# lux-liang/Robust-Audio-Deepfake-Evolution

Measured on AMD Instinct MI355X. Metric: Phase-6 train throughput (utterances/sec), DualStreamSEMamba + LoRA + RawBoost/codec + FGM, higher is better.
Workload: dtype fp16; 1 GPU; Phase6_Proposed.conf train step on ASVspoof19-LA-shaped utterances; micro_batch=8, accumulation=4, global_batch=32, seq_len=64600, parallelism=dp1, fgm=True, mixup=True, rawboost_algo=5, lora_mode=reference, hip_graphs=True, window_batched_clean_passes=True

## Files before the change

### include/radhip.h

```cpp
#ifndef RADHIP_H
#define RADHIP_H

#include <stdint.h>

#ifdef __cplusplus
extern "C" {
#endif

#define RDX_OK 0
#define RDX_EINVAL (-1)
#define RDX_EUNSUPPORTED (-2)

typedef enum { RDX_F32 = 0, RDX_BF16 = 1 } rdx_dtype;

const char* rdx_version(void);
const char* rdx_strerror(int code);

int rdx_sincconv_absmaxpool_fwd(const float* x, int64_t batch, int64_t len, const float* filters,
                                int channels, int ksize, int mask_lo, int mask_hi, float* out,
                                void* stream);
int rdx_sincconv_absmaxpool_fwd_devmask(const float* x, int64_t batch, int64_t len,
                                        const float* filters, int channels, int ksize,
                                        const int32_t* mask_dev, int mask_stride, float* out,
                                        void* stream);
int rdx_sincconv_absmaxpool_f16mfma(const float* x, int64_t batch, int64_t len, const float* filters, int channels,
                                    int ksize, int mask_lo, int mask_hi, const int32_t* mask_dev, int mask_stride,
                                    float* out, void* stream);
int rdx_sincconv_abspool1d_fwd(const float* x, int64_t batch, int64_t len, const float* filters,
                               int channels, int ksize, int mask_lo, int mask_hi, float* out, void* stream);


int rdx_dwconv_bidir_fwd(int dtype, const void* x, int64_t ldx, const float* w, const float* bias,
                         void* u, int B, int L, int D, int K, int dirs, void* stream);
int rdx_dwconv_bidir_bwd_parts(int L);
int rdx_dwconv_bidir_bwd(int dtype, const void* x, int64_t ldx, const float* w, const float* bias,
                         const void* du, void* dx, int64_t lddx, float* dw_part, float* db_part, int64_t ld_part,
                         int B, int L, int D, int K, int dirs, void* stream);

int64_t rdx_scan_ckpt_elems(int B, int L, int D, int N, int dirs);
int rdx_scan_nblk_d(int D);
int rdx_selective_scan_fwd(int dtype, const void* u, const void* delta, const float* A_log,
                           const void* Bm, const void* Cm, int64_t ldbc, const float* Dp,
                           const float* dt_bias, float* y, float* ckpt, int B, int L, int D, int N,
                           int dirs, void* stream);
int rdx_selective_scan_bwd(int dtype, const void* u, const void* delta, const float* A_log,
                           const void* Bm, const void* Cm, int64_t ldbc, const float* Dp,
                           const float* dt_bias, const float* ckpt, const float* dy,
                           int64_t dy_dir_stride, void* du, void* ddelta, float* dBC,
                           float* dA_part, float* dD_part, float* dbias_part, int B, int L, int D,
                           int N, int dirs, void* stream);

int rdx_bigate_fwd(int dtype, const float* y, int dirs, const void* z, int64_t ldz, void* g,
                   float* ysum, int B, int L, int D, void* stream);
int rdx_bigate_bwd(int dtype, const void* dg, const void* z, int64_t ldz, const float* ysum,
                   float* dy, void* dz, int64_t lddz, int B, int L, int D, void* stream);

int rdx_row_ln_fwd(int dtype_x, const void* x, const float* gamma, const float* beta, float eps, int dtype_y, void* y,
                   float* mean, float* rstd, int64_t M, int C, void* stream);
int rdx_row_ln_bwd(int dtype_dy, const void* dy, int dtype_x, const void* x, const float* mean, const float* rstd,
                   const float* gamma, void* dx, float* dgamma, float* dbeta, int64_t M, int C, void* stream);

int rdx_layer_wsum_fwd(int dtype, int nl, const void* const* hs, const float* w, void* out,
                       int64_t n, void* stream);
int rdx_layer_wsum_nblk(int64_t n);
int rdx_layer_wsum_bwd(int dtype, int nl, const void* const* hs, const float* w, const void* g,
                       void* const* dhs, float* dot_part, int64_t n, void* stream);
int rdx_cast_f32_many(int n, const float* const* src, void* const* dst, const int64_t* numel, void* stream);
int rdx_add_f32_many(int n, void* const* dst, const float* const* src, const int64_t* numel, int copy, void* stream);

typedef struct {
  int64_t offset;
  int64_t len;
  int32_t algo;
  int32_t n_a;
  double b[6];
  double a[6];
  double f;
  double beta;
  double snr_db;
  uint64_t seed;
} rdx_rawboost_utt;

int64_t rdx_rawboost_workspace_bytes(int nutt, int64_t total_samples);
int rdx_rawboost_batch(const float* x, float* out, const rdx_rawboost_utt* utts, int nutt,
                       void* workspace, const double* noise_isd, const double* noise_ssi,
                       void* stream);

int rdx_resample_kernel(int orig_freq, int new_freq, int lowpass_width, double rolloff,
                        float* host_kernel, int host_kernel_cap, int* width_out, int* orig_g_out,
                        int* new_g_out);
typedef struct {
  int64_t in_offset, in_len, out_offset, out_len;
  int32_t orig_g, new_g, width, kern_offset;
} rdx_resample_job;
int rdx_resample_batch(const float* in, float* out, const float* kernels,
                       const rdx_resample_job* jobs, int njobs, void* stream);

int rdx_pad_mixup(const float* sig, const int64_t* offsets, const int64_t* lens,
                  const int64_t* starts, int nutt, int64_t max_len, const int* perm, float lam,
                  float* out, void* stream);

int rdx_fgm_attack(int ntensors, float* const* params, const float* const* grads,
                   float* const* backup, const int64_t* numels, float eps, double* workspace,
                   void* stream);

int rdx_focal_mixup_fwd(const void* logits, int logits_bf16, int ld, int B, int C, const int64_t* ya,
                        const int64_t* yb, const float* lam, int rows_per_lam, float alpha, float gamma,
                        int mode, float scale, float* loss, float* dlogits, void* stream);
int rdx_focal_mixup_bwd(const float* grad, const float* dlogits, void* out, int out_bf16, int n, void* stream);

int rdx_ocsupcon_eligible(const void* feats, int ld, int R, int D, int B);
int rdx_ocsupcon_mixup_fwd(const void* feats, int feats_bf16, int ld, int R, int D, const float* center,
                           const int64_t* ya, const int64_t* yb, const float* lam, int rows_per_lam,
                           float r_real, float r_fake, float alpha, float lambda_supcon, float temperature,
                           float base_temperature, float scale, float* loss, float* loss_parts, float* dfeats,
                           float* dcenter_parts, void* stream);
int rdx_ocsupcon_mixup_bwd(const float* grad, const float* dfeats, void* out, int out_bf16, int64_t n,
                           const float* dcenter_parts, int K, int D, float* dcenter, void* stream);

int rdx_gat_eligible(const void* x, int N, int Din, int Dout, float temp);
int rdx_gat_att_fwd(const float* x, const float* W, const float* b, const float* w, float temp, int B, int N,
                    int Din, int Dout, float* att, float* agg, void* stream);
int rdx_gat_att_bwd(const float* dagg, const float* x, const float* W, const float* b, const float* w, float temp,
                    const float* att, int B, int N, int Din, int Dout, float* dx, float* dW, float* db, float* dw,
                    void* stream);

int rdx_bnselu_fwd(int dtype, const void* c, const float* conv_bias, const float* mean, const float* invstd,
                   const float* weight, const float* bias, void* y, int64_t npix, int C, void* stream);
int rdx_bnselu_bwd(int dtype, const void* c, const void* dy, const float* conv_bias, const float* mean,
                   const float* invstd, const float* weight, const float* bias, void* dc, float* sums,
                   int64_t npix, int C, void* stream);
int rdx_res_tail_fwd(int dtype, const void* a, const void* identity, const float* bias, void* y,
                     uint8_t* argmax, int64_t rows, int W, int C, void* stream);
int rdx_res_tail_bwd(int dtype, const void* dy, const uint8_t* argmax, void* dx, float* dbias, int64_t rows,
                     int W, int C, void* stream);
int rdx_sincnet_b0_fwd(const void* x, const float* w1, const float* wd, const float* bn, void* c, void* y, void* idn,
                       int N, int H, int W, int C, void* stream);
int rdx_sincnet_b0_nblk(int64_t npix);
int rdx_b0x_fwd(const void* x, const float* w1, const float* wd, const float* bn, const void* w2, const float* bias,
                void* y, uint8_t* arg, int N, int H, int W, void* stream);
int rdx_b0x_bwd_nblk(int N, int W);
int rdx_b0x_bwd(const void* x, const void* dp, const uint8_t* arg, const float* w1, const float* wd, const float* bn,
                const void* w2f, float* dx, float* part, int N, int H, int W, void* stream);
int rdx_sincnet_b0_bwd(const void* x, const void* dc, const void* di, const float* w1, const float* wd, float* dx,
                       float* part, int N, int H, int W, int C, void* stream);

int rdx_posconv_fwd(const void* h, const void* wk, const float* bias, void* y, void* u, int B, int T, void* stream);
int rdx_posconv_bwd(const void* dy, const void* u, const void* wkt, void* dh, int B, int T, void* stream);

int rdx_attn_fwd(const void* q, int64_t ldq, const void* k, int64_t ldk, const void* v, int64_t ldv,
                 const float* gate, const float* rel_bias, const int64_t* seed_dev, int salt, float p_drop,
                 float scale, void* o, int64_t ldo, float* lse, uint32_t* keep_mask, int B, int T, int H, int head_dim,
                 void* stream);
int64_t rdx_attn_keep_mask_words(int B, int T, int H);
int rdx_attn_bwd(const void* q, int64_t ldq, const void* k, int64_t ldk, const void* v, int64_t ldv,
                 const float* gate, const float* rel_bias, const int64_t* seed_dev, int salt, float p_drop, float scale,
                 const void* o, int64_t ldo, const float* lse, const void* dout, int64_t lddo, float* D, void* dq,
                 void* dk, void* dv, int64_t ldg, float* dgate, int B, int T, int H, int head_dim, void* stream);
int rdx_attn_bwd_fused(const void* q, int64_t ldq, const void* k, int64_t ldk, const void* v, int64_t ldv,
                       const float* gate, const float* rel_bias, const uint32_t* keep_mask, float p_drop, float scale,
                       const void* o, int64_t ldo, const float* lse, const void* dout, int64_t lddo, float* D,
                       void* dq, void* dk, void* dv, int64_t ldg, float* dgate, int B, int T, int H, int head_dim,
                       void* stream);
int64_t rdx_attn_bwd_split_ws(int B, int H);
int rdx_attn_bwd_fused_split(const void* q, int64_t ldq, const void* k, int64_t ldk, const void* v, int64_t ldv,
                             const float* gate, const float* rel_bias, const uint32_t* keep_mask, float p_drop,
                             float scale, const void* o, int64_t ldo, const float* lse, const void* dout,
                             int64_t lddo, float* D, void* dq, void* dk, void* dv, int64_t ldg, float* dgate,
                             float* ws, int64_t ws_floats, int* counters, int64_t n_counters, int B, int T, int H,
                             int head_dim, void* stream);
int rdx_attn_dropout_mask(const int64_t* seed_dev, int salt, float p_drop, uint8_t* keep, int64_t n, int T,
                          void* stream);
int rdx_dropout_mask(const int64_t* seed_dev, int salt, float p_drop, uint8_t* keep, int64_t n, void* stream);

int rdx_wl_ln1_fwd(const float* h, const float* gamma, const float* beta, float eps, const float* wg,
                   const float* bg, const float* gconst, const void* lora_aq, const void* lora_av, int r,
                   const int64_t* seed_dev, int salt_q, int salt_v, float p_lora, void* x1, int64_t ldx, float* gate, float* mean,
                   float* rstd, int64_t M, int E, void* stream);
int rdx_wl_add_ln_fwd(const float* h, const void* delta, const int64_t* seed_dev, int salt, float p, float* h2,
                      const float* gamma, const float* beta, float eps, void* x, float* mean, float* rstd,
                      int64_t M, int E, void* stream);
int rdx_wl_residual(const float* h, const void* delta, const int64_t* seed_dev, int salt, float p, float* out,
                    int64_t n, void* stream);
int rdx_wl_dropout_bwd(const float* g, const int64_t* seed_dev, int salt, float p, void* out, int64_t n,
                       void* stream);
int rdx_wl_gelu(int mode, const void* u, const void* dy, void* out, int64_t n, void* stream);
int rdx_wl_ln_bwd(const void* dx, int64_t ldd, const float* h, const float* mean, const float* rstd,
                  const float* gamma, const float* dres, float* dh, const int64_t* seed_dev, int salt, float p,
                  void* ddrop, int64_t M, int E, void* stream);
int rdx_wl_ln1_bwd(const void* dx1, int64_t ldx, const float* dgate, const float* h, const float* mean,
                   const float* rstd, const float* gamma, const float* beta, const float* wg, const float* bg,
                   const float* gconst, const void* lora_aq, const void* lora_av, int r,
                   const int64_t* seed_dev, int salt_q, int salt_v, float p_lora, const float* dres, float* dh, void* xd, int64_t M, int E,
                   void* stream);
int rdx_wl_res_ln1_fwd(const float* h2, const void* delta, int salt_res, float p_res, float* hout,
                       const float* gamma, const float* beta, float eps, const float* wg, const float* bg,
                       const float* gconst, const void* lora_aq, const void* lora_av, int r, const int64_t* seed_dev,
                       int salt_q, int salt_v, float p_lora, void* x1, int64_t ldx, float* gate, float* mean,
                       float* rstd, int64_t M, int E, void* stream);
int rdx_wl_ln1_bwd_ex(const void* dx1, int64_t ldx, const float* dgate, const float* h, const float* mean,
                      const float* rstd, const float* gamma, const float* beta, const float* wg, const float* bg,
                      const float* gconst, const void* lora_aq, const void* lora_av, int r, const int64_t* seed_dev,
                      int salt_q, int salt_v, float p_lora, const float* dres, float* dh, void* xd,
                      const float* state_grad, const float* state_weight, int salt_prev, float p_prev,
                      void* ddrop_prev, int64_t M, int E, void* stream);
int rdx_wl_lora_grad(const void* dqkv, int64_t ldq, const void* x1, int64_t ldx, const void* dx1, int64_t ldd,
                     const int64_t* seed_dev, int salt_q, int salt_v, float p_lora, float scale, float* daq,
                     float* dbq, float* dav, float* dbv, int64_t M, int E, int r, void* stream);
int rdx_wl_lora_pack(int nl, const float* const* bq, const float* const* bv, void* const* wext, int64_t ldw,
                     int r, float scale, int E, void* stream);

#define RDX_EPI_BIAS 0
#define RDX_EPI_BIAS_GELU 1
#define RDX_EPI_GELU_BWD 2
#define RDX_EPI_RESID_DROP 3
int rdx_gemm_bf16(const void* A, int64_t lda, const void* B, int64_t ldb, void* C, int64_t ldc, int M, int N, int K,
                  const void* bias, int epilogue, const void* aux, int64_t ldaux, void* aux_out, int64_t ldao,
                  const int64_t* seed_dev, int salt, float p_drop, void* stream);

int rdx_scan2_chunks(int L);
int64_t rdx_scan2_rec_elems(int B, int L, int D, int N, int dirs);
int rdx_scan2_fwd(int dtype, const void* u, const void* delta, const float* A_log, const void* Bm, const void* Cm,
                  int64_t ldbc, const float* Dp, const float* dt_bias, float* y, float* ckpt, float* P, float* hloc,
                  int B, int L, int D, int N, int dirs, void* stream);
int rdx_scan2_bwd(int dtype, const void* u, const void* delta, const float* A_log, const void* Bm, const void* Cm,
                  int64_t ldbc, const float* Dp, const float* dt_bias, const float* ckpt, const float* P,
                  const float* dy, int64_t dy_dir_stride, void* du, void* ddelta, float* dBC, float* dA_part,
                  float* dD_part, float* dbias_part, int64_t ld_part, float* gloc, int B, int L, int D, int N,
                  int dirs, void* stream);

int rdx_wgemm_bf16(const void* A, int64_t lda, const void* B, int64_t ldb, void* C, int64_t ldc, int M, int N, int K,
                   const void* bias, int epilogue, const void* aux, int64_t ldaux, void* aux_out, int64_t ldao,
                   int tile, void* stream);
int rdx_wgemm_pick(int M, int N, int K);
int rdx_wgemm_bf16_ex(const void* A, int64_t lda, const void* B, int64_t ldb, void* C, int64_t ldc, int M, int N,
                      int K, const void* bias, int epilogue, const void* aux, int64_t ldaux, void* aux_out,
                      int64_t ldao, int tile, int splits, void* ws, int64_t ws_bytes, int* counters,
                      int64_t n_counters, void* stream);
int64_t rdx_wgemm_ws_bytes(int M, int N, int tile, int splits);
int64_t rdx_wgemm_counters(int M, int N, int tile);

int rdx_pgemm_bf16(const void* A, int64_t lda, const void* B, int64_t ldb, void* C, int64_t ldc, int M, int N, int K,
                   const void* bias, int epilogue, const void* aux, int64_t ldaux, void* aux_out, int64_t ldao,
                   int tile, int group_m, void* stream);
int rdx_pgemm_prof(const void* A, int64_t lda, const void* B, int64_t ldb, void* C, int64_t ldc, int M, int N, int K,
                   const void* bias, int tile, int group_m, void* prof, void* stream);

int rdx_hgemm(const void* A, int64_t lda, const void* B, int64_t ldb, void* C, int64_t ldc, int M, int N, int K,
              const void* bias, int epilogue, const void* aux, int64_t ldaux, void* aux_out, int64_t ldao, int tile,
              int splits, int group_m, void* ws, int64_t ws_bytes, int* counters, int64_t n_counters, void* stream);
int64_t rdx_hgemm_ws_bytes(int M, int N, int tile, int splits);
int64_t rdx_hgemm_counters(int M, int N, int tile);
int64_t rdx_hgemm_sk_ws_bytes(int M, int N, int K, int tile);
int rdx_hgemm_batched(const void* A, int64_t lda, int64_t sa, const void* B, int64_t ldb, void* C, int64_t ldc,
                      int64_t sc, int M, int N, int K, int batch, const void* bias, int tile, int group_m, void* stream);

#define RDX_EPI_F32 4
#define RDX_EPI_F32_GELU_SPLIT 5
int rdx_hgemm_x3(const void* A, const void* A_lo, int64_t lda, int64_t sa, const void* B, const void* B_lo,
                 int64_t ldb, void* C, void* C_lo, int64_t ldc, int64_t sc, int M, int N, int K, int batch,
                 const float* bias, int epilogue, int tile, int splits, int group_m, void* ws, int64_t ws_bytes,
                 int* counters, int64_t n_counters, void* stream);

int rdx_x3_split(const float* x, int64_t ldx, int64_t rows, int cols, void* hi, void* lo, int64_t ldo, void* stream);
int rdx_x3_ln_split(const float* a, const float* b, float* sum_out, const float* gamma, const float* beta, float eps,
                    void* hi, void* lo, int64_t ldo, float* y32, const float* wg, const float* bg, const float* gconst,
                    float* gate, int64_t M, int E, void* stream);
int rdx_x3_attn_fwd(const float* q, const float* k, const float* v, int64_t ld, const float* gate, const float* rel,
                    float scaling, void* ohi, void* olo, int64_t ldo, int B, int T, int H, int qsplit, void* stream);
int rdx_x3_posconv_fwd(const float* h, const void* wk_hi, const void* wk_lo, const float* bias, float* out, int B,
                       int T, void* stream);
int rdx_x3_fe_conv0(const float* x, int64_t batch, int64_t len, const float* w, const float* bias, const float* gamma,
                    const float* beta, float eps, int ksize, int stride, void* out_hi, void* out_lo, void* stream);
int rdx_x3_fe_ln_gelu(const float* in, int64_t rows, const float* bias, const float* gamma, const float* beta,
                      float eps, void* out_hi, void* out_lo, float* out32, void* stream);

int rdx_x3_b0x_fwd(const float* x, const float* fbn, const float* w1, const float* wd, const float* bn,
                   const void* w2_hi, const void* w2_lo, const float* bias, float* y, int N, int H, int W,
                   void* stream);
int rdx_x3_sconv_fwd(const float* x, const void* w_hi, const void* w_lo, const float* bn, float* y, int N, int H,
                     int W, int ci, int co, int kh, int ph, void* stream);

int rdx_colsum_many(int n, const float* const* in, const int* rows, const int* cols, const int64_t* ld,
                    float* const* out, void* stream);

int rdx_lgemm(const void* A, int64_t lda, int a_f32, const void* W, int64_t ldw, void* C, int64_t ldc, int c_f32,
              int M, int N, int K, const void* bias, int epilogue, const void* aux, int64_t ldaux, void* aux_out,
              int64_t ldao, const void* R, int64_t ldr, void* stream);

int rdx_wgrad_chunk(int M, int N, int K);
int64_t rdx_wgrad_ws_floats(int M, int N, int K);
int rdx_wgrad_acc(const void* dy, int64_t ldy, const void* x, int64_t ldx, int M, int N, int K, float* dw, int64_t ldw,
                  float* db, float* ws, int64_t ws_floats, void* stream);
int64_t rdx_wgrad_many_ws_floats(int n, const int* M, const int* N, const int* K, const int* has_db);
int rdx_wgrad_acc_many(int n, const void* const* dy, const int64_t* ldy, const void* const* x, const int64_t* ldx,
                       const int* M, const int* N, const int* K, float* const* dw, const int64_t* ldw,
                       float* const* db, float* ws, int64_t ws_floats, void* stream);

int rdx_adamw_many_max(void);
int rdx_adamw_many(int n, float* const* params, float* const* grads, float* const* exp_avg, float* const* exp_avg_sq,
                   const float* const* step, const int64_t* numel, double lr, double beta1, double beta2,
                   double weight_decay, double eps, const float* grad_scale, const float* found_inf, void* stream);

int rdx_timestamp_acc(int64_t* acc, int sign, void* stream);
int rdx_wallclock_khz(int device);

int rdx_gemm_bf16_strided(const void* A, int64_t lda, int64_t sA, const void* B, int64_t ldb, void* C, int64_t ldc,
                          int64_t crow, int batch, int M, int N, int K, const void* bias, void* stream);

int rdx_fe_conv0(const float* x, int64_t batch, int64_t len, const float* w, const float* bias, const float* gamma,
                 const float* beta, float eps, int ksize, int stride, void* out, void* stream);
int rdx_fe_ln_gelu(void* io, int64_t rows, const float* gamma, const float* beta, float eps, float* out32,
                   void* stream);

int rdx_sconv_fwd(const void* x, const void* w, void* y, void* y2, const float* bn, int N, int H, int W, int ci,
                  int co, int kh, int ph, void* stream);
int rdx_sconv_fwd_res(const void* x, const void* w, void* y, const void* res, int N, int H, int W, int ci, int co,
                      int kh, int ph, void* stream);
int rdx_sconv_dgrad_bnselu(const void* dy, const void* w, const void* c, void* dc, const float* bn, float* sums,
                           int N, int H, int W, int ci, int co, int kh, int ph, void* stream);
int rdx_sconv_fwd_pool(const void* x, const void* w, const void* idn, const float* bias, void* y, uint8_t* arg, int N,
                       int H, int W, int ci, int co, void* stream);
int rdx_sconv_fwd_res_pool(const void* x, const void* w, void* y, const void* dp, const uint8_t* arg, float* dbias,
                           int N, int H, int W, int ci, int co, int kh, int ph, void* stream);
int rdx_sconv_dgrad_bnselu_pool(const void* dp, const uint8_t* arg, const void* w, const void* c, void* dc,
                                const float* bn, float* sums, int N, int H, int W, int ci, int co, int kh, int ph,
                                void* stream);
int rdx_sconv_dgrad_pool(const void* dp, const uint8_t* arg, const void* w, void* dx, int N, int H, int W, int ci,
                         int co, int kh, int ph, void* stream);
int rdx_sconv_wgrad_pool(const void* x, const void* dp, const uint8_t* arg, float* dw, float* part, int N, int H,
                         int W, int ci, int co, int kh, int ph, void* stream);
int rdx_sconv_wgrad_nblk(int N, int Ho, int W);
int rdx_sconv_wgrad(const void* x, const void* dy, float* dw, float* part, int N, int H, int W, int ci, int co,
                    int kh, int ph, void* stream);
int rdx_se_fwd(const void* x, const void* w1, const void* w2, void* y, void* m, void* h, void* s, int B, int T, int C,
               int R, void* stream);
int64_t rdx_se_bwd_part_floats(int B, int C, int R);
int rdx_se_bwd(const void* dy, const void* x, const void* w1, const void* w2, const void* m, const void* h, const void* s,
               void* dx, float* part, float* dw1, float* dw2, int B, int T, int C, int R, void* stream);
int rdx_attn_pool_fwd(const void* f, const void* w, const void* bias, void* feat, float* a, int B, int T, int C,
                      void* stream);
int rdx_attn_pool_bwd(const void* f, const void* w, const float* a, const void* dfeat, void* df, float* part, float* dw,
                      float* db, int B, int T, int C, void* stream);
int rdx_upcat_fwd(const void* fw, const void* fs, void* out, int B, int T1, int T2, int C, void* stream);
int rdx_upcat_bwd(const void* dout, void* dfs, int B, int T1, int T2, int C, void* stream);
int rdx_sconv_wprep_many(int n, const float* const* src, void* const* wf, void* const* wd, const int* co,
                         const int* ci, const int* kh, void* stream);

#ifdef __cplusplus
}
#endif
#endif
```

### robust-audio-deepfake-evolution_amd/csrc/wavlm_layer.hip

```cpp
#include "common.h"

namespace rdx {

constexpr int WL_E = 1024;
constexpr int WL_VPL = WL_E / RDX_WAVE;
constexpr int WL_R2 = 16;

struct Drop {
  const int64_t* seed_dev;
  int salt;
  uint32_t thr;
  float inv_keep;
};

__device__ __forceinline__ float drop_scale(const Drop& d, uint64_t seed, uint64_t idx) {
  return drop_keep(seed, idx, d.thr) ? d.inv_keep : 0.f;
}

__device__ __forceinline__ void load16(const float* p, float* v) {
  const float4* q = reinterpret_cast<const float4*>(p);
#pragma unroll
  for (int i = 0; i < 4; ++i) {
    float4 t = q[i];
    v[4 * i] = t.x; v[4 * i + 1] = t.y; v[4 * i + 2] = t.z; v[4 * i + 3] = t.w;
  }
}
__device__ __forceinline__ void store16(float* p, const float* v) {
  float4* q = reinterpret_cast<float4*>(p);
#pragma unroll
  for (int i = 0; i < 4; ++i) q[i] = make_float4(v[4 * i], v[4 * i + 1], v[4 * i + 2], v[4 * i + 3]);
}
__device__ __forceinline__ void load16_bf(const hst* p, float* v) {
  const uint4* q = reinterpret_cast<const uint4*>(p);
#pragma unroll
  for (int i = 0; i < 2; ++i) {
    uint4 t = q[i];
    uint32_t w[4] = {t.x, t.y, t.z, t.w};
#pragma unroll
    for (int j = 0; j < 4; ++j) {
      v[8 * i + 2 * j] = hlo(w[j]);
      v[8 * i + 2 * j + 1] = hhi(w[j]);
    }
  }
}
struct Bf16x16 {
  uint4 q[2];
};
__device__ __forceinline__ Bf16x16 load16_bf_raw(const hst* p) {
  const uint4* q = reinterpret_cast<const uint4*>(p);
  return Bf16x16{{q[0], q[1]}};
}
__device__ __forceinline__ void unpack16_bf(const Bf16x16& t, float* v) {
#pragma unroll
  for (int i = 0; i < 2; ++i) {
    uint32_t w[4] = {t.q[i].x, t.q[i].y, t.q[i].z, t.q[i].w};
#pragma unroll
    for (int j = 0; j < 4; ++j) {
      v[8 * i + 2 * j] = hlo(w[j]);
      v[8 * i + 2 * j + 1] = hhi(w[j]);
    }
  }
}
__device__ __forceinline__ void store16_bf(hst* p, const float* v) {
  uint4* q = reinterpret_cast<uint4*>(p);
#pragma unroll
  for (int i = 0; i < 2; ++i) {
    uint32_t w[4];
#pragma unroll
    for (int j = 0; j < 4; ++j) w[j] = hbits(v[8 * i + 2 * j]) | (hbits(v[8 * i + 2 * j + 1]) << 16);
    q[i] = make_uint4(w[0], w[1], w[2], w[3]);
  }
}

__device__ __forceinline__ void row_stats(const float* v, float eps, float& mean, float& rstd) {
  float s = 0.f;
#pragma unroll
  for (int i = 0; i < WL_VPL; ++i) s += v[i];
  mean = wave_sum(s) * (1.0f / WL_E);
  float q = 0.f;
#pragma unroll
  for (int i = 0; i < WL_VPL; ++i) {
    float d = v[i] - mean;
    q += d * d;
  }
  rstd = rsqrtf(wave_sum(q) * (1.0f / WL_E) + eps);
}

__device__ __forceinline__ float wave_sum16(float* v, int lane) {
  float w8[8], w4[4], w2[2];
  const bool h5 = lane & 32, h4 = lane & 16, h3 = lane & 8, h2 = lane & 4;
#pragma unroll
  for (int j = 0; j < 8; ++j) {
    float r = __shfl_xor(h5 ? v[j] : v[j + 8], 32, 64);
    w8[j] = (h5 ? v[j + 8] : v[j]) + r;
  }
#pragma unroll
  for (int j = 0; j < 4; ++j) {
    float r = __shfl_xor(h4 ? w8[j] : w8[j + 4], 16, 64);
    w4[j] = (h4 ? w8[j + 4] : w8[j]) + r;
  }
#pragma unroll
  for (int j = 0; j < 2; ++j) {
    float r = __shfl_xor(h3 ? w4[j] : w4[j + 2], 8, 64);
    w2[j] = (h3 ? w4[j + 2] : w4[j]) + r;
  }
  float r = __shfl_xor(h2 ? w2[0] : w2[1], 4, 64);
  float t = (h2 ? w2[1] : w2[0]) + r;
  t += __shfl_xor(t, 2, 64);
  t += __shfl_xor(t, 1, 64);
  return t;
}
__device__ __forceinline__ int sum16_index(int lane) {
  return 8 * ((lane >> 5) & 1) + 4 * ((lane >> 4) & 1) + 2 * ((lane >> 3) & 1) + ((lane >> 2) & 1);
}

struct GateW {
  const float* wg;
  const float* bg;
  const float* gconst;
};

__device__ __forceinline__ void gate_z(const GateW& g, const float* wgp, const float* x, int lane, float* z) {
  const int part = lane & 3;
#pragma unroll
  for (int j = 0; j < 8; ++j) {
    const float4* w = reinterpret_cast<const float4*>(wgp + j * 64 + part * 16);
    float acc = 0.f;
#pragma unroll
    for (int i = 0; i < 4; ++i) {
      float4 t = w[i];
      acc += t.x * x[4 * i] + t.y * x[4 * i + 1] + t.z * x[4 * i + 2] + t.w * x[4 * i + 3];
    }
    acc += __shfl_xor(acc, 1, 64);
    acc += __shfl_xor(acc, 2, 64);
    z[j] = acc + g.bg[j];
  }
}

struct Ln1Args {
  const float* h;
  const float* gamma;
  const float* beta;
  float eps;
  GateW g;
  const hst* Aq;
  const hst* Av;
  Drop dq, dv;
  hst* x1;
  int64_t ldx;
  float* gate;
  float* mean;
  float* rstd;
  int64_t M;
  const float* h2;
  const hst* delta;
  Drop dres;
  float* hout;
};

#ifndef WL_LN1_ROWS_DEF
#define WL_LN1_ROWS_DEF 4
#endif
constexpr int WL_LN1_ROWS = WL_LN1_ROWS_DEF;
constexpr int WL_LN1_THREADS = WL_LN1_ROWS * RDX_WAVE;

typedef __attribute__((ext_vector_type(4))) int wl_i32x4;
__device__ void wl_load_lds(wl_i32x4 rsrc, __attribute__((address_space(3))) uint32_t* lds, int size, int voffset,
                            int soffset, int offset, int aux) __asm("llvm.amdgcn.raw.buffer.load.lds");
__device__ __forceinline__ wl_i32x4 wl_rsrc(const void* base, uint32_t bytes) {
  const uint64_t a = (uint64_t)base;
  wl_i32x4 r;
  r.x = (int)(uint32_t)a;
  r.y = (int)(uint32_t)(a >> 32);
  r.z = (int)bytes;
  r.w = 0x00020000;
  return r;
}
constexpr int WL_A_INSTR = WL_R2 * WL_E * 2 / 1024 / (WL_LN1_THREADS / 64);
static_assert(WL_A_INSTR * 1024 * (WL_LN1_THREADS / 64) == WL_R2 * WL_E * 2, "whole 1 KB instructions per wave");
template <bool kLora>
__device__ __forceinline__ void stage_dma(float* swg, hst* sA, const float* wg, const hst* Aq, const hst* Av) {
  const int wv = __builtin_amdgcn_readfirstlane(threadIdx.x >> 6), lane = threadIdx.x & 63;
  constexpr int NW = WL_LN1_THREADS / 64;
  if (wv == 0) {
    const wl_i32x4 rg = wl_rsrc(wg, 8 * 64 * 4);
#pragma unroll
    for (int q = 0; q < 2; ++q)
      wl_load_lds(rg, (__attribute__((address_space(3))) uint32_t*)(reinterpret_cast<char*>(swg) + 1024 * q), 16,
                  1024 * q + 16 * lane, 0, 0, 0);
  }
  if (kLora) {
    const wl_i32x4 rq = wl_rsrc(Aq, WL_R2 / 2 * WL_E * 2), rv = wl_rsrc(Av, WL_R2 / 2 * WL_E * 2);
#pragma unroll
    for (int j = 0; j < WL_A_INSTR; ++j) {
      const int q = wv + NW * j;
      constexpr int half = WL_R2 / 2 * WL_E * 2 / 1024;
      wl_load_lds(j < WL_A_INSTR / 2 ? rq : rv,
                  (__attribute__((address_space(3))) uint32_t*)(reinterpret_cast<char*>(sA) + 1024 * q), 16,
                  1024 * (q % half) + 16 * lane, 0, 0, 0);
    }
  }
}

template <bool kLora>
__global__ __launch_bounds__(WL_LN1_THREADS) void wl_ln1_fwd_kernel(Ln1Args a) {
  __shared__ __attribute__((aligned(16))) hst sA[kLora ? WL_R2 * WL_E : 8];
  __shared__ __attribute__((aligned(16))) float swg[8 * 64];
  const int lane = threadIdx.x & 63;
  const int64_t m = (int64_t)blockIdx.x * WL_LN1_ROWS + (threadIdx.x >> 6);
  const bool live = m < a.M;
  const int e0 = lane * WL_VPL;
  float v[WL_VPL], gm[WL_VPL], bt[WL_VPL], dl[WL_VPL];
  Bf16x16 dlr;
  const uint64_t sr = (a.h2 && a.dres.thr) ? attn_seed(a.dres.seed_dev, a.dres.salt) : 0;
  stage_dma<kLora>(swg, sA, a.g.wg, a.Aq, a.Av);
  if (live) {
    load16(a.h2 ? a.h2 + m * WL_E + e0 : a.h + m * WL_E + e0, v);
    if (a.h2) dlr = load16_bf_raw(a.delta + m * WL_E + e0);
    load16(a.gamma + e0, gm);
    load16(a.beta + e0, bt);
  }
  __builtin_amdgcn_s_waitcnt(0);
  __syncthreads();
  if (live) {
    if (a.h2) {
      unpack16_bf(dlr, dl);

#pragma unroll
      for (int i = 0; i < WL_VPL; ++i)
        v[i] += dl[i] * (a.dres.thr ? drop_scale(a.dres, sr, (uint64_t)m * WL_E + e0 + i) : 1.0f);
      store16(a.hout + m * WL_E + e0, v);
    }
    float mean, rstd;
    row_stats(v, a.eps, mean, rstd);
#pragma unroll
    for (int i = 0; i < WL_VPL; ++i) v[i] = hround((v[i] - mean) * rstd * gm[i] + bt[i]);
    store16_bf(a.x1 + m * a.ldx + e0, v);
    if (lane == 0) {
      a.mean[m] = mean;
      a.rstd[m] = rstd;
    }
    float z[8];
    gate_z(a.g, swg, v, lane, z);
    if ((lane & 3) == 0) {
      const int head = lane >> 2;
      float ga = sigmoidf_(z[0] + z[1] + z[2] + z[3]);
      float gb = sigmoidf_(z[4] + z[5] + z[6] + z[7]);
      a.gate[m * (WL_E / 64) + head] = ga * (gb * a.g.gconst[head] - 1.0f) + 2.0f;
    }
  }
  if (kLora) {
    if (!live) return;
    const uint64_t sq = a.dq.thr ? attn_seed(a.dq.seed_dev, a.dq.salt) : 0;
    const uint64_t sv = a.dv.thr ? attn_seed(a.dv.seed_dev, a.dv.salt) : 0;
    uint32_t mq[WL_VPL / 2], mv[WL_VPL / 2];
#pragma unroll
    for (int j = 0; j < WL_VPL / 2; ++j) {
      const uint64_t idx = (uint64_t)m * WL_E + e0 + 2 * j;
      mq[j] = hpack2(v[2 * j] * drop_scale(a.dq, sq, idx), v[2 * j + 1] * drop_scale(a.dq, sq, idx + 1));
      mv[j] = hpack2(v[2 * j] * drop_scale(a.dv, sv, idx), v[2 * j + 1] * drop_scale(a.dv, sv, idx + 1));
    }
    float acc[WL_R2];
#pragma unroll
    for (int k = 0; k < WL_R2; ++k) {
      const uint32_t* x = k < WL_R2 / 2 ? mq : mv;
      const uint4* wp = reinterpret_cast<const uint4*>(sA + k * WL_E + e0);
      const uint4 w0 = wp[0], w1 = wp[1];
      const uint32_t w[8] = {w0.x, w0.y, w0.z, w0.w, w1.x, w1.y, w1.z, w1.w};
      float s = 0.f;
#pragma unroll
      for (int j = 0; j < WL_VPL / 2; ++j) s = hdot2(w[j], x[j], s);
      acc[k] = s;
    }
    float tot = wave_sum16(acc, lane);
    if ((lane & 3) == 0) a.x1[m * a.ldx + WL_E + sum16_index(lane)] = f2h(tot);
  }
}

struct AddLnArgs {
  const float* h;
  const hst* delta;
  Drop d;
  float* h2;
  const float* gamma;
  const float* beta;
  float eps;
  hst* x;
  float* mean;
  float* rstd;
  int64_t M;
};

__global__ __launch_bounds__(256) void wl_add_ln_fwd_kernel(AddLnArgs a) {
  const int lane = threadIdx.x & 63;
  const int64_t m = (int64_t)blockIdx.x * 4 + (threadIdx.x >> 6);
  if (m >= a.M) return;
  const int e0 = lane * WL_VPL;
  float v[WL_VPL], dl[WL_VPL], gm[WL_VPL], bt[WL_VPL];
  load16(a.h + m * WL_E + e0, v);
  const Bf16x16 dlr = load16_bf_raw(a.delta + m * WL_E + e0);
  load16(a.gamma + e0, gm);
  load16(a.beta + e0, bt);
  unpack16_bf(dlr, dl);
  const uint64_t seed = a.d.thr ? attn_seed(a.d.seed_dev, a.d.salt) : 0;
#pragma unroll
  for (int i = 0; i < WL_VPL; ++i)
    v[i] += dl[i] * (a.d.thr ? drop_scale(a.d, seed, (uint64_t)m * WL_E + e0 + i) : 1.0f);
  store16(a.h2 + m * WL_E + e0, v);
  float mean, rstd;
  row_stats(v, a.eps, mean, rstd);
#pragma unroll
  for (int i = 0; i < WL_VPL; ++i) v[i] = (v[i] - mean) * rstd * gm[i] + bt[i];
  store16_bf(a.x + m * WL_E + e0, v);
  if (lane == 0) {
    a.mean[m] = mean;
    a.rstd[m] = rstd;
  }
}

__global__ __launch_bounds__(256) void wl_residual_kernel(const float* __restrict__ h,
                                                          const hst* __restrict__ delta, Drop d,
                                                          float* __restrict__ out, int64_t n) {
  const int64_t i0 = ((int64_t)blockIdx.x * 256 + threadIdx.x) * 8;
  if (i0 >= n) return;
  const uint64_t seed = d.thr ? attn_seed(d.seed_dev, d.salt) : 0;
  float4 a0 = reinterpret_cast<const float4*>(h + i0)[0], a1 = reinterpret_cast<const float4*>(h + i0)[1];
  float x[8] = {a0.x, a0.y, a0.z, a0.w, a1.x, a1.y, a1.z, a1.w};
  uint4 t = *reinterpret_cast<const uint4*>(delta + i0);
  uint32_t w[4] = {t.x, t.y, t.z, t.w};
#pragma unroll
  for (int j = 0; j < 8; ++j) {
    float dv = (j & 1) ? hhi(w[j >> 1]) : hlo(w[j >> 1]);
    x[j] += dv * (d.thr ? drop_scale(d, seed, (uint64_t)(i0 + j)) : 1.0f);
  }
  reinterpret_cast<float4*>(out + i0)[0] = make_float4(x[0], x[1], x[2], x[3]);
  reinterpret_cast<float4*>(out + i0)[1] = make_float4(x[4], x[5], x[6], x[7]);
}

__global__ __launch_bounds__(256) void wl_dropout_bwd_kernel(const float* __restrict__ g, Drop d,
                                                             hst* __restrict__ out, int64_t n) {
  const int64_t i0 = ((int64_t)blockIdx.x * 256 + threadIdx.x) * 8;
  if (i0 >= n) return;
  const uint64_t seed = d.thr ? attn_seed(d.seed_dev, d.salt) : 0;
  float4 a0 = reinterpret_cast<const float4*>(g + i0)[0], a1 = reinterpret_cast<const float4*>(g + i0)[1];
  float x[8] = {a0.x, a0.y, a0.z, a0.w, a1.x, a1.y, a1.z, a1.w};
  uint32_t w[4];
#pragma unroll
  for (int j = 0; j < 4; ++j) {
    float s0 = d.thr ? drop_scale(d, seed, (uint64_t)(i0 + 2 * j)) : 1.0f;
    float s1 = d.thr ? drop_scale(d, seed, (uint64_t)(i0 + 2 * j + 1)) : 1.0f;
    w[j] = hbits(x[2 * j] * s0) | (hbits(x[2 * j + 1] * s1) << 16);
  }
  *reinterpret_cast<uint4*>(out + i0) = make_uint4(w[0], w[1], w[2], w[3]);
}

__device__ __forceinline__ float gelu_erf(float x) { return 0.5f * x * (1.0f + erff(x * 0.70710678118654752f)); }
__device__ __forceinline__ float gelu_erf_grad(float x) {
  return 0.5f * (1.0f + erff(x * 0.70710678118654752f)) + x * 0.39894228040143268f * __expf(-0.5f * x * x);
}

template <int kMode>
__global__ __launch_bounds__(256) void wl_gelu_kernel(const hst* __restrict__ u,
                                                      const hst* __restrict__ dy,
                                                      hst* __restrict__ out, int64_t n) {
  const int64_t i0 = ((int64_t)blockIdx.x * 256 + threadIdx.x) * 8;
  if (i0 >= n) return;
  uint4 t = *reinterpret_cast<const uint4*>(u + i0);
  uint32_t w[4] = {t.x, t.y, t.z, t.w}, gw[4] = {0, 0, 0, 0};
  if (kMode == 1) {
    uint4 g = *reinterpret_cast<const uint4*>(dy + i0);
    gw[0] = g.x; gw[1] = g.y; gw[2] = g.z; gw[3] = g.w;
  }
  uint32_t o[4];
#pragma unroll
  for (int j = 0; j < 4; ++j) {
    float x0 = hlo(w[j]), x1 = hhi(w[j]);
    float y0, y1;
    if (kMode == 0) {
      y0 = gelu_erf(x0);
      y1 = gelu_erf(x1);
    } else {
      y0 = hlo(gw[j]) * gelu_erf_grad(x0);
      y1 = hhi(gw[j]) * gelu_erf_grad(x1);
    }
    o[j] = hbits(y0) | (hbits(y1) << 16);
  }
  *reinterpret_cast<uint4*>(out + i0) = make_uint4(o[0], o[1], o[2], o[3]);
}

struct LnBwdArgs {
  const hst* dx;
  int64_t ldd;
  const float* h;
  const float* mean;
  const float* rstd;
  const float* gamma;
  const float* dres;
  float* dh;
  Drop d;
  hst* ddrop;
  int64_t M;
};

__device__ __forceinline__ void ln_bwd_row(const float* dx, const float* x, float mean, float rstd, const float* gm,
                                           float* out) {
  float g[WL_VPL], xh[WL_VPL], s1 = 0.f, s2 = 0.f;
#pragma unroll
  for (int i = 0; i < WL_VPL; ++i) {
    xh[i] = (x[i] - mean) * rstd;
    g[i] = dx[i] * gm[i];
    s1 += g[i];
    s2 += g[i] * xh[i];
  }
  s1 = wave_sum(s1) * (1.0f / WL_E);
  s2 = wave_sum(s2) * (1.0f / WL_E);
#pragma unroll
  for (int i = 0; i < WL_VPL; ++i) out[i] = rstd * (g[i] - s1 - xh[i] * s2);
}

__global__ __launch_bounds__(256) void wl_ln_bwd_kernel(LnBwdArgs a) {
  const int lane = threadIdx.x & 63;
  const int64_t m = (int64_t)blockIdx.x * 4 + (threadIdx.x >> 6);
  if (m >= a.M) return;
  const int e0 = lane * WL_VPL;
  float dx[WL_VPL], x[WL_VPL], gm[WL_VPL], o[WL_VPL], r[WL_VPL];
  const uint64_t seed = (a.ddrop && a.d.thr) ? attn_seed(a.d.seed_dev, a.d.salt) : 0;
  const Bf16x16 dxr = load16_bf_raw(a.dx + m * a.ldd + e0);
  load16(a.h + m * WL_E + e0, x);
  load16(a.gamma + e0, gm);
  if (a.dres) load16(a.dres + m * WL_E + e0, r);
  unpack16_bf(dxr, dx);
  ln_bwd_row(dx, x, a.mean[m], a.rstd[m], gm, o);
  if (a.dres) {
#pragma unroll
    for (int i = 0; i < WL_VPL; ++i) o[i] += r[i];
  }
  store16(a.dh + m * WL_E + e0, o);
  if (a.ddrop) {
#pragma unroll
    for (int i = 0; i < WL_VPL; ++i)
      o[i] *= a.d.thr ? drop_scale(a.d, seed, (uint64_t)m * WL_E + e0 + i) : 1.0f;
    store16_bf(a.ddrop + m * WL_E + e0, o);
  }
}

struct Ln1BwdArgs {
  const hst* dx1;
  int64_t ldx;
  const float* dgate;
  const float* h;
  const float* mean;
  const float* rstd;
  const float* gamma;
  const float* beta;
  GateW g;
  const hst* Aq;
  const hst* Av;
  Drop dq, dv;
  const float* dres;
  float* dh;
  hst* xd;
  int64_t M;
  const float* sg;
  const float* sw;
  Drop dprev;
  hst* ddrop;
};

template <bool kLora>
__global__ __launch_bounds__(WL_LN1_THREADS) void wl_ln1_bwd_kernel(Ln1BwdArgs a) {
  __shared__ __attribute__((aligned(16))) hst sA[kLora ? WL_R2 * WL_E : 8];
  __shared__ __attribute__((aligned(16))) float swg[8 * 64];
  const int lane = threadIdx.x & 63;
  const int64_t m = (int64_t)blockIdx.x * WL_LN1_ROWS + (threadIdx.x >> 6);
  const bool live = m < a.M;
  const int e0 = lane * WL_VPL;
  const int part = lane & 3, head = lane >> 2;
  float x[WL_VPL], x1[WL_VPL], dx[WL_VPL], r[WL_VPL], sgv[WL_VPL], gm[WL_VPL];
  float mean = 0.f, rstd = 0.f, dg = 0.f;
  Bf16x16 dxr;
  const uint64_t sp = (a.ddrop && a.dprev.thr) ? attn_seed(a.dprev.seed_dev, a.dprev.salt) : 0;
  stage_dma<kLora>(swg, sA, a.g.wg, a.Aq, a.Av);
  if (live) {
    load16(a.h + m * WL_E + e0, x);
    dxr = load16_bf_raw(a.dx1 + m * a.ldx + e0);
    load16(a.dres + m * WL_E + e0, r);
    if (a.sg) load16(a.sg + m * WL_E + e0, sgv);
    load16(a.gamma + e0, gm);
    load16(a.beta + e0, x1);
    mean = a.mean[m];
    rstd = a.rstd[m];
    dg = a.dgate[m * (WL_E / 64) + head];
  }
  __builtin_amdgcn_s_waitcnt(0);
  __syncthreads();
  if (!live) return;
  unpack16_bf(dxr, dx);
#pragma unroll
  for (int i = 0; i < WL_VPL; ++i) x1[i] = hround((x[i] - mean) * rstd * gm[i] + x1[i]);
  float z[8];
  gate_z(a.g, swg, x1, lane, z);
  const float ga = sigmoidf_(z[0] + z[1] + z[2] + z[3]), gb = sigmoidf_(z[4] + z[5] + z[6] + z[7]);
  const float c = a.g.gconst[head];
  const float dza = dg * (gb * c - 1.0f) * ga * (1.0f - ga);
  const float dzb = dg * ga * c * gb * (1.0f - gb);
#pragma unroll 2
  for (int j = 0; j < 8; ++j) {
    const float dz = j < 4 ? dza : dzb;
    const float4* w = reinterpret_cast<const float4*>(swg + j * 64 + part * 16);
#pragma unroll
    for (int i = 0; i < 4; ++i) {
      float4 t = w[i];
      dx[4 * i] += t.x * dz;
      dx[4 * i + 1] += t.y * dz;
      dx[4 * i + 2] += t.z * dz;
      dx[4 * i + 3] += t.w * dz;
    }
  }
  if (kLora) {
    const uint64_t sq = a.dq.thr ? attn_seed(a.dq.seed_dev, a.dq.salt) : 0;
    const uint64_t sv = a.dv.thr ? attn_seed(a.dv.seed_dev, a.dv.salt) : 0;
    if (a.xd) {
#pragma unroll
      for (int which = 0; which < 2; ++which) {
        const Drop& dd = which ? a.dv : a.dq;
        const uint64_t sd = which ? sv : sq;
        float xm[WL_VPL];
#pragma unroll
        for (int i = 0; i < WL_VPL; ++i) xm[i] = x1[i] * drop_scale(dd, sd, (uint64_t)m * WL_E + e0 + i);
        store16_bf(a.xd + (which * a.M + m) * WL_E + e0, xm);
      }
    }
    const uint4 dap[2] = {*reinterpret_cast<const uint4*>(a.dx1 + m * a.ldx + WL_E),
                          *reinterpret_cast<const uint4*>(a.dx1 + m * a.ldx + WL_E + 8)};
#pragma unroll
    for (int which = 0; which < 2; ++which) {
      float acc[WL_VPL];
#pragma unroll
      for (int i = 0; i < WL_VPL; ++i) acc[i] = 0.f;
      const uint32_t dk[4] = {dap[which].x, dap[which].y, dap[which].z, dap[which].w};
#pragma unroll
      for (int kp = 0; kp < WL_R2 / 4; ++kp) {
        const int k = which * (WL_R2 / 2) + 2 * kp;
        const uint4* ra = reinterpret_cast<const uint4*>(sA + k * WL_E + e0);
        const uint4* rb = reinterpret_cast<const uint4*>(sA + (k + 1) * WL_E + e0);
        const uint4 a0 = ra[0], a1 = ra[1], b0 = rb[0], b1 = rb[1];
        const uint32_t wa[8] = {a0.x, a0.y, a0.z, a0.w, a1.x, a1.y, a1.z, a1.w};
        const uint32_t wb[8] = {b0.x, b0.y, b0.z, b0.w, b1.x, b1.y, b1.z, b1.w};
#pragma unroll
        for (int j = 0; j < WL_VPL / 2; ++j) {
          const uint32_t ev = __builtin_amdgcn_perm(wb[j], wa[j], 0x05040100u);
          const uint32_t od = __builtin_amdgcn_perm(wb[j], wa[j], 0x07060302u);
          acc[2 * j] = hdot2(ev, dk[kp], acc[2 * j]);
          acc[2 * j + 1] = hdot2(od, dk[kp], acc[2 * j + 1]);
        }
      }
      const Drop& dd = which ? a.dv : a.dq;
      const uint64_t sd = which ? sv : sq;
#pragma unroll
      for (int i = 0; i < WL_VPL; ++i) dx[i] += acc[i] * drop_scale(dd, sd, (uint64_t)m * WL_E + e0 + i);
    }
  }
  float o[WL_VPL];
  ln_bwd_row(dx, x, mean, rstd, gm, o);
#pragma unroll
  for (int i = 0; i < WL_VPL; ++i) o[i] += r[i];
  if (a.sg) {
    const float pw = a.sw[0];
#pragma unroll
    for (int i = 0; i < WL_VPL; ++i) o[i] = fmaf(pw, sgv[i], o[i]);
  }
  store16(a.dh + m * WL_E + e0, o);
  if (a.ddrop) {
#pragma unroll
    for (int i = 0; i < WL_VPL; ++i)
      o[i] *= a.dprev.thr ? drop_scale(a.dprev, sp, (uint64_t)m * WL_E + e0 + i) : 1.0f;
    store16_bf(a.ddrop + m * WL_E + e0, o);
  }
}

constexpr int WL_LG_COLS = 128;
constexpr int WL_LG_PAD = WL_LG_COLS + 1;

struct LoraGradArgs {
  const hst* dqkv;
  int64_t ldq;
  const hst* x1;
  int64_t ldx;
  const hst* dx1;
  int64_t ldd;
  Drop dq, dv;
  float scale;
  float *dAq, *dBq, *dAv, *dBv;
  int64_t M;
};

__device__ __forceinline__ float2 hx2_at(const hst* p) {
  const uint32_t u = *reinterpret_cast<const uint32_t*>(p);
  return make_float2(hlo(u), hhi(u));
}

template <int RPW>
__global__ __launch_bounds__(256, 2) void wl_lora_grad_kernel(LoraGradArgs a, int nch) {
  constexpr int ROWS = 4 * RPW;
  __shared__ float s_row[2][ROWS][2 * WL_R2];
  __shared__ float s_part[4][2 * WL_R2][WL_LG_PAD];
  const int lane = threadIdx.x & 63, w = threadIdx.x >> 6;
  const int e0 = blockIdx.x * WL_LG_COLS;
  const int e = e0 + 2 * lane;
  constexpr int R = WL_R2 / 2;
  float bq[2][R], bv[2][R], aq[2][R], av[2][R];
#pragma unroll
  for (int c = 0; c < 2; ++c)
#pragma unroll
    for (int k = 0; k < R; ++k) bq[c][k] = bv[c][k] = aq[c][k] = av[c][k] = 0.f;
  const uint64_t sq = a.dq.thr ? attn_seed(a.dq.seed_dev, a.dq.salt) : 0;
  const uint64_t sv = a.dv.thr ? attn_seed(a.dv.seed_dev, a.dv.salt) : 0;
  for (int ch = 0; ch < nch; ++ch) {
    const int64_t m0 = ((int64_t)blockIdx.y * nch + ch) * ROWS;
    float(*srow)[2 * WL_R2] = s_row[ch & 1];
    for (int t = threadIdx.x; t < ROWS * 2 * WL_R2; t += 256) {
      const int rr = t / (2 * WL_R2), c = t % (2 * WL_R2);
      const int64_t m = m0 + rr;
      float v = 0.f;
      if (m < a.M)
        v = c < WL_R2 ? h2f(a.x1[m * a.ldx + WL_E + c])
                      : h2f(a.dx1[m * a.ldd + WL_E + c - WL_R2]);
      srow[rr][c] = v;
    }
    float2 gq[RPW], gv[RPW], xx[RPW];
#pragma unroll
    for (int j = 0; j < RPW; ++j) {
      const int64_t m = min(m0 + w * RPW + j, a.M - 1);
      gq[j] = hx2_at(a.dqkv + m * a.ldq + e);
      gv[j] = hx2_at(a.dqkv + m * a.ldq + 2 * WL_E + e);
      xx[j] = hx2_at(a.x1 + m * a.ldx + e);
    }
    __syncthreads();
#pragma unroll
    for (int j = 0; j < RPW; ++j) {
      const int rr = w * RPW + j;
      const uint64_t idx = (uint64_t)min(m0 + rr, a.M - 1) * WL_E + e;
      const float g_q[2] = {gq[j].x, gq[j].y}, g_v[2] = {gv[j].x, gv[j].y};
      const float xq[2] = {xx[j].x * drop_scale(a.dq, sq, idx), xx[j].y * drop_scale(a.dq, sq, idx + 1)};
      const float xv[2] = {xx[j].x * drop_scale(a.dv, sv, idx), xx[j].y * drop_scale(a.dv, sv, idx + 1)};
      const float* f = srow[rr];
#pragma unroll
      for (int c = 0; c < 2; ++c)
#pragma unroll
        for (int k = 0; k < R; ++k) {
          bq[c][k] = fmaf(g_q[c], f[k], bq[c][k]);
          bv[c][k] = fmaf(g_v[c], f[R + k], bv[c][k]);
          aq[c][k] = fmaf(f[2 * R + k], xq[c], aq[c][k]);
          av[c][k] = fmaf(f[3 * R + k], xv[c], av[c][k]);
        }
    }
  }
#pragma unroll
  for (int c = 0; c < 2; ++c)
#pragma unroll
    for (int k = 0; k < R; ++k) {
      s_part[w][k][2 * lane + c] = bq[c][k];
      s_part[w][R + k][2 * lane + c] = bv[c][k];
      s_part[w][2 * R + k][2 * lane + c] = aq[c][k];
      s_part[w][3 * R + k][2 * lane + c] = av[c][k];
    }
  __syncthreads();
#pragma unroll 4
  for (int i = 0; i < 16; ++i) {
    const int o = i * 256 + threadIdx.x;
    int row, col;
    float* dst;
    float mul = 1.f;
    if (o < 2048) {
      const int kk = o / WL_LG_COLS;
      col = o % WL_LG_COLS;
      row = 2 * R + kk;
      dst = kk < R ? a.dAq + (int64_t)kk * WL_E + e0 + col : a.dAv + (int64_t)(kk - R) * WL_E + e0 + col;
    } else {
      const int o2 = o - 2048, which = o2 / (WL_LG_COLS * R), rem = o2 % (WL_LG_COLS * R);
      col = rem / R;
      const int k = rem % R;
      row = which * R + k;
      dst = (which ? a.dBv : a.dBq) + (int64_t)(e0 + col) * R + k;
      mul = a.scale;
    }
    const float v = s_part[0][row][col] + s_part[1][row][col] + s_part[2][row][col] + s_part[3][row][col];
    atomicAdd(dst, mul * v);
  }
}

__global__ __launch_bounds__(256) void wl_lora_pack_kernel(int nl, const float* const* bq, const float* const* bv,
                                                           hst* const* wext, int64_t ldw, int r,
                                                           float scale) {
  const int l = blockIdx.y;
  const int64_t t = (int64_t)blockIdx.x * 256 + threadIdx.x;
  if (l >= nl || t >= 2 * (int64_t)WL_E * r) return;
  const int which = (int)(t / ((int64_t)WL_E * r));
  const int64_t rem = t % ((int64_t)WL_E * r);
  const int64_t row = rem / r;
  const int k = (int)(rem % r);
  const float* b = which ? bv[l] : bq[l];
  const int64_t wrow = which ? 2 * WL_E + row : row;
  wext[l][wrow * ldw + WL_E + which * r + k] = f2h(scale * b[row * r + k]);
}

}

using namespace rdx;

static Drop mk_drop(const int64_t* seed_dev, int salt, float p) {
  Drop d;
  d.seed_dev = seed_dev;
  d.salt = salt;
  d.thr = (p > 0.f && seed_dev) ? (uint32_t)fminf(4294967295.0f, p * 4294967296.0f) : 0u;
  d.inv_keep = p > 0.f ? 1.0f / (1.0f - p) : 1.0f;
  return d;
}

static int blocks_rows(int64_t M) { return (int)((M + 3) / 4); }
static int blocks_ln1(int64_t M) { return (int)((M + WL_LN1_ROWS - 1) / WL_LN1_ROWS); }

static int ln1_fwd_launch(const Ln1Args& a, bool lora, void* stream) {
  const int64_t M = a.M;
  if (lora)
    hipLaunchKernelGGL(wl_ln1_fwd_kernel<true>, dim3(blocks_ln1(M)), dim3(WL_LN1_THREADS), 0, as_stream(stream), a);
  else
    hipLaunchKernelGGL(wl_ln1_fwd_kernel<false>, dim3(blocks_ln1(M)), dim3(WL_LN1_THREADS), 0, as_stream(stream), a);
  RDX_LAUNCH_CHECK();
  return 0;
}


extern "C" {

int rdx_wl_ln1_fwd(const float* h, const float* gamma, const float* beta, float eps, const float* wg, const float* bg,
                   const float* gconst, const void* lora_aq, const void* lora_av, int r, const int64_t* seed_dev,
                   int salt_q, int salt_v, float p_lora, void* x1, int64_t ldx, float* gate, float* mean, float* rstd, int64_t M, int E,
                   void* stream) {
  RDX_REQUIRE(h && gamma && beta && wg && bg && gconst && x1 && gate && mean && rstd && M > 0);
  const bool lora = lora_aq != nullptr;
  RDX_REQUIRE(E == WL_E && (!lora || (2 * r == WL_R2 && lora_av)) && ldx >= E + (lora ? 2 * r : 0));
  RDX_REQUIRE(!lora || ((((uintptr_t)lora_aq | (uintptr_t)lora_av) & 15) == 0));
  RDX_REQUIRE(ldx % 8 == 0);
  Ln1Args a{h, gamma, beta, eps, GateW{wg, bg, gconst}, reinterpret_cast<const hst*>(lora_aq),
            reinterpret_cast<const hst*>(lora_av), mk_drop(seed_dev, salt_q, p_lora),
            mk_drop(seed_dev, salt_v, p_lora), reinterpret_cast<hst*>(x1), ldx, gate, mean, rstd, M,
            nullptr, nullptr, mk_drop(nullptr, 0, 0.f), nullptr};
  return ln1_fwd_launch(a, lora, stream);
}

int rdx_wl_res_ln1_fwd(const float* h2, const void* delta, int salt_res, float p_res, float* hout,
                       const float* gamma, const float* beta, float eps, const float* wg, const float* bg,
                       const float* gconst, const void* lora_aq, const void* lora_av, int r, const int64_t* seed_dev,
                       int salt_q, int salt_v, float p_lora, void* x1, int64_t ldx, float* gate, float* mean,
                       float* rstd, int64_t M, int E, void* stream) {
  RDX_REQUIRE(h2 && delta && hout && gamma && beta && wg && bg && gconst && x1 && gate && mean && rstd && M > 0);
  const bool lora = lora_aq != nullptr;
  RDX_REQUIRE(E == WL_E && (!lora || (2 * r == WL_R2 && lora_av)) && ldx >= E + (lora ? 2 * r : 0));
  RDX_REQUIRE(!lora || ((((uintptr_t)lora_aq | (uintptr_t)lora_av) & 15) == 0));
  RDX_REQUIRE(ldx % 8 == 0);
  Ln1Args a{nullptr, gamma, beta, eps, GateW{wg, bg, gconst}, reinterpret_cast<const hst*>(lora_aq),
            reinterpret_cast<const hst*>(lora_av), mk_drop(seed_dev, salt_q, p_lora),
            mk_drop(seed_dev, salt_v, p_lora), reinterpret_cast<hst*>(x1), ldx, gate, mean, rstd, M,
            h2, reinterpret_cast<const hst*>(delta), mk_drop(seed_dev, salt_res, p_res), hout};
  return ln1_fwd_launch(a, lora, stream);
}

int rdx_wl_add_ln_fwd(const float* h, const void* delta, const int64_t* seed_dev, int salt, float p, float* h2,
                      const float* gamma, const float* beta, float eps, void* x, float* mean, float* rstd, int64_t M,
                      int E, void* stream) {
  RDX_REQUIRE(h && delta && h2 && gamma && beta && x && mean && rstd && M > 0 && E == WL_E);
  AddLnArgs a{h, reinterpret_cast<const hst*>(delta), mk_drop(seed_dev, salt, p), h2, gamma, beta, eps,
              reinterpret_cast<hst*>(x), mean, rstd, M};
  hipLaunchKernelGGL(wl_add_ln_fwd_kernel, dim3(blocks_rows(M)), dim3(256), 0, as_stream(stream), a);
  RDX_LAUNCH_CHECK();
  return 0;
}

int rdx_wl_residual(const float* h, const void* delta, const int64_t* seed_dev, int salt, float p, float* out,
                    int64_t n, void* stream) {
  RDX_REQUIRE(h && delta && out && n > 0 && n % 8 == 0);
  hipLaunchKernelGGL(wl_residual_kernel, dim3((unsigned)((n / 8 + 255) / 256)), dim3(256), 0, as_stream(stream), h,
                     reinterpret_cast<const hst*>(delta), mk_drop(seed_dev, salt, p), out, n);
  RDX_LAUNCH_CHECK();
  return 0;
}

int rdx_wl_dropout_bwd(const float* g, const int64_t* seed_dev, int salt, float p, void* out, int64_t n,
                       void* stream) {
  RDX_REQUIRE(g && out && n > 0 && n % 8 == 0);
  hipLaunchKernelGGL(wl_dropout_bwd_kernel, dim3((unsigned)((n / 8 + 255) / 256)), dim3(256), 0, as_stream(stream), g,
                     mk_drop(seed_dev, salt, p), reinterpret_cast<hst*>(out), n);
  RDX_LAUNCH_CHECK();
  return 0;
}

int rdx_wl_gelu(int mode, const void* u, const void* dy, void* out, int64_t n, void* stream) {
  RDX_REQUIRE(u && out && n > 0 && n % 8 == 0 && (mode == 0 || (mode == 1 && dy)));
  const auto* U = reinterpret_cast<const hst*>(u);
  const auto* DY = reinterpret_cast<const hst*>(dy);
  auto* O = reinterpret_cast<hst*>(out);
  const dim3 grid((unsigned)((n / 8 + 255) / 256));
  if (mode == 0)
    hipLaunchKernelGGL(wl_gelu_kernel<0>, grid, dim3(256), 0, as_stream(stream), U, DY, O, n);
  else
    hipLaunchKernelGGL(wl_gelu_kernel<1>, grid, dim3(256), 0, as_stream(stream), U, DY, O, n);
  RDX_LAUNCH_CHECK();
  return 0;
}

int rdx_wl_ln_bwd(const void* dx, int64_t ldd, const float* h, const float* mean, const float* rstd,
                  const float* gamma, const float* dres, float* dh, const int64_t* seed_dev, int salt, float p,
                  void* ddrop, int64_t M, int E, void* stream) {
  RDX_REQUIRE(dx && h && mean && rstd && gamma && dh && M > 0 && E == WL_E && ldd >= E && ldd % 8 == 0);
  LnBwdArgs a{reinterpret_cast<const hst*>(dx), ldd, h, mean, rstd, gamma, dres, dh,
              mk_drop(seed_dev, salt, p), reinterpret_cast<hst*>(ddrop), M};
  hipLaunchKernelGGL(wl_ln_bwd_kernel, dim3(blocks_rows(M)), dim3(256), 0, as_stream(stream), a);
  RDX_LAUNCH_CHECK();
  return 0;
}

int rdx_wl_ln1_bwd_ex(const void* dx1, int64_t ldx, const float* dgate, const float* h, const float* mean,
                      const float* rstd, const float* gamma, const float* beta, const float* wg, const float* bg,
                      const float* gconst, const void* lora_aq, const void* lora_av, int r, const int64_t* seed_dev,
                      int salt_q, int salt_v, float p_lora, const float* dres, float* dh, void* xd,
                      const float* state_grad, const float* state_weight, int salt_prev, float p_prev,
                      void* ddrop_prev, int64_t M, int E, void* stream) {
  RDX_REQUIRE(dx1 && dgate && h && mean && rstd && gamma && beta && wg && bg && gconst && dres && dh && M > 0);
  RDX_REQUIRE((state_grad == nullptr) == (state_weight == nullptr));
  const bool lora = lora_aq != nullptr;
  RDX_REQUIRE(E == WL_E && ldx % 8 == 0 && (!lora || (2 * r == WL_R2 && lora_av && ldx >= E + 2 * r)));
  RDX_REQUIRE(!lora || ((((uintptr_t)lora_aq | (uintptr_t)lora_av) & 15) == 0));
  Ln1BwdArgs a{reinterpret_cast<const hst*>(dx1), ldx, dgate, h, mean, rstd, gamma, beta,
               GateW{wg, bg, gconst}, reinterpret_cast<const hst*>(lora_aq), reinterpret_cast<const hst*>(lora_av),
               mk_drop(seed_dev, salt_q, p_lora), mk_drop(seed_dev, salt_v, p_lora),
               dres, dh, reinterpret_cast<hst*>(xd), M, state_grad, state_weight,
               mk_drop(seed_dev, salt_prev, p_prev), reinterpret_cast<hst*>(ddrop_prev)};
  if (lora)
    hipLaunchKernelGGL(wl_ln1_bwd_kernel<true>, dim3(blocks_ln1(M)), dim3(WL_LN1_THREADS), 0, as_stream(stream), a);
  else
    hipLaunchKernelGGL(wl_ln1_bwd_kernel<false>, dim3(blocks_ln1(M)), dim3(WL_LN1_THREADS), 0, as_stream(stream), a);
  RDX_LAUNCH_CHECK();
  return 0;
}

int rdx_wl_ln1_bwd(const void* dx1, int64_t ldx, const float* dgate, const float* h, const float* mean,
                   const float* rstd, const float* gamma, const float* beta, const float* wg, const float* bg,
                   const float* gconst, const void* lora_aq, const void* lora_av, int r, const int64_t* seed_dev,
                   int salt_q, int salt_v, float p_lora, const float* dres, float* dh, void* xd, int64_t M, int E,
                   void* stream) {
  return rdx_wl_ln1_bwd_ex(dx1, ldx, dgate, h, mean, rstd, gamma, beta, wg, bg, gconst, lora_aq, lora_av, r, seed_dev,
                           salt_q, salt_v, p_lora, dres, dh, xd, nullptr, nullptr, 0, 0.f, nullptr, M, E, stream);
}

int rdx_wl_lora_grad(const void* dqkv, int64_t ldq, const void* x1, int64_t ldx, const void* dx1, int64_t ldd,
                     const int64_t* seed_dev, int salt_q, int salt_v, float p_lora, float scale, float* daq,
                     float* dbq, float* dav, float* dbv, int64_t M, int E, int r, void* stream) {
  RDX_REQUIRE(dqkv && x1 && dx1 && daq && dbq && dav && dbv && M > 0 && E == WL_E && 2 * r == WL_R2);
  RDX_REQUIRE(ldq >= 3 * (int64_t)E && ldx >= E + 2 * r && ldd >= E + 2 * r);
  RDX_REQUIRE(ldq % 2 == 0 && ldx % 2 == 0 && ((uintptr_t)dqkv & 3) == 0 && ((uintptr_t)x1 & 3) == 0);
  LoraGradArgs a{reinterpret_cast<const hst*>(dqkv), ldq, reinterpret_cast<const hst*>(x1), ldx,
                 reinterpret_cast<const hst*>(dx1), ldd, mk_drop(seed_dev, salt_q, p_lora),
                 mk_drop(seed_dev, salt_v, p_lora), scale, daq, dbq, dav, dbv, M};
  const int64_t nchunk = (M + 31) / 32;
  const int nch = (int)std::max<int64_t>(1, std::min<int64_t>(8, M / 2048));
  const dim3 grid(WL_E / WL_LG_COLS, (unsigned)((nchunk + nch - 1) / nch));
  hipLaunchKernelGGL(wl_lora_grad_kernel<8>, grid, dim3(256), 0, as_stream(stream), a, nch);
  RDX_LAUNCH_CHECK();
  return 0;
}

int rdx_wl_lora_pack(int nl, const float* const* bq, const float* const* bv, void* const* wext, int64_t ldw, int r,
                     float scale, int E, void* stream) {
  RDX_REQUIRE(nl > 0 && bq && bv && wext && E == WL_E && r > 0 && ldw >= E + 2 * r);
  const int64_t n = 2 * (int64_t)E * r;
  hipLaunchKernelGGL(wl_lora_pack_kernel, dim3((unsigned)((n + 255) / 256), nl), dim3(256), 0, as_stream(stream), nl,
                     bq, bv, reinterpret_cast<hst* const*>(wext), ldw, r, scale);
  RDX_LAUNCH_CHECK();
  return 0;
}

}
```

### robust-audio-deepfake-evolution_amd/radhip/_lib.py

```python
import ctypes
import os
import threading

_HERE = os.path.dirname(os.path.abspath(__file__))
LIB_PATH = os.environ.get("RADHIP_LIB", os.path.join(_HERE, "libradhip.so"))
LIB16_PATH = os.environ.get("RADHIP_LIB16", os.path.join(_HERE, "libradhip_f16.so"))

RDX_F32 = 0
RDX_BF16 = 1
EPI_BIAS, EPI_BIAS_GELU, EPI_GELU_BWD, EPI_RESID_DROP = 0, 1, 2, 3
EPI_F32, EPI_F32_GELU_SPLIT = 4, 5

c_int = ctypes.c_int
c_i64 = ctypes.c_int64
c_f32 = ctypes.c_float
c_f64 = ctypes.c_double
c_vp = ctypes.c_void_p
c_fp = ctypes.c_void_p


class RawboostUtt(ctypes.Structure):

    _fields_ = [
        ("offset", c_i64),
        ("len", c_i64),
        ("algo", ctypes.c_int32),
        ("n_a", ctypes.c_int32),
        ("b", c_f64 * 6),
        ("a", c_f64 * 6),
        ("f", c_f64),
        ("beta", c_f64),
        ("snr_db", c_f64),
        ("seed", ctypes.c_uint64),
    ]


class ResampleJob(ctypes.Structure):

    _fields_ = [
        ("in_offset", c_i64),
        ("in_len", c_i64),
        ("out_offset", c_i64),
        ("out_len", c_i64),
        ("orig_g", ctypes.c_int32),
        ("new_g", ctypes.c_int32),
        ("width", ctypes.c_int32),
        ("kern_offset", ctypes.c_int32),
    ]


SIGNATURES = {
    "rdx_version": (ctypes.c_char_p, []),
    "rdx_strerror": (ctypes.c_char_p, [c_int]),
    "rdx_sincconv_absmaxpool_fwd": (c_int, [c_vp, c_i64, c_i64, c_vp, c_int, c_int, c_int, c_int, c_vp, c_vp]),
    "rdx_sincconv_abspool1d_fwd": (c_int, [c_vp, c_i64, c_i64, c_vp, c_int, c_int, c_int, c_int, c_vp, c_vp]),
    "rdx_sincconv_absmaxpool_fwd_devmask": (c_int, [c_vp, c_i64, c_i64, c_vp, c_int, c_int, c_vp, c_int, c_vp,
                                                    c_vp]),
    "rdx_dwconv_bidir_fwd": (c_int, [c_int, c_vp, c_i64, c_vp, c_vp, c_vp, c_int, c_int, c_int, c_int, c_int, c_vp]),
    "rdx_dwconv_bidir_bwd_parts": (c_int, [c_int]),
    "rdx_dwconv_bidir_bwd": (c_int, [c_int, c_vp, c_i64, c_vp, c_vp, c_vp, c_vp, c_i64, c_vp, c_vp, c_i64,
                                     c_int, c_int, c_int, c_int, c_int, c_vp]),
    "rdx_scan_ckpt_elems": (c_i64, [c_int, c_int, c_int, c_int, c_int]),
    "rdx_scan_nblk_d": (c_int, [c_int]),
    "rdx_selective_scan_fwd": (c_int, [c_int, c_vp, c_vp, c_vp, c_vp, c_vp, c_i64, c_vp, c_vp, c_vp, c_vp,
                                       c_int, c_int, c_int, c_int, c_int, c_vp]),
    "rdx_selective_scan_bwd": (c_int, [c_int, c_vp, c_vp, c_vp, c_vp, c_vp, c_i64, c_vp, c_vp, c_vp, c_vp, c_i64,
                                       c_vp, c_vp, c_vp, c_vp, c_vp, c_vp, c_int, c_int, c_int, c_int, c_int, c_vp]),
    "rdx_bigate_fwd": (c_int, [c_int, c_vp, c_int, c_vp, c_i64, c_vp, c_vp, c_int, c_int, c_int, c_vp]),
    "rdx_bigate_bwd": (c_int, [c_int, c_vp, c_vp, c_i64, c_vp, c_vp, c_vp, c_i64, c_int, c_int, c_int, c_vp]),
    "rdx_layer_wsum_fwd": (c_int, [c_int, c_int, ctypes.POINTER(c_vp), c_vp, c_vp, c_i64, c_vp]),
    "rdx_layer_wsum_nblk": (c_int, [c_i64]),
    "rdx_cast_f32_many": (c_int, [c_int, ctypes.POINTER(c_vp), ctypes.POINTER(c_vp), ctypes.POINTER(c_i64), c_vp]),
    "rdx_add_f32_many": (c_int, [c_int, ctypes.POINTER(c_vp), ctypes.POINTER(c_vp), ctypes.POINTER(c_i64), c_int,
                                 c_vp]),
    "rdx_layer_wsum_bwd": (c_int, [c_int, c_int, ctypes.POINTER(c_vp), c_vp, c_vp, ctypes.POINTER(c_vp), c_vp,
                                   c_i64, c_vp]),
    "rdx_rawboost_workspace_bytes": (c_i64, [c_int, c_i64]),
    "rdx_rawboost_batch": (c_int, [c_vp, c_vp, ctypes.POINTER(RawboostUtt), c_int, c_vp, c_vp, c_vp, c_vp]),
    "rdx_resample_kernel": (c_int, [c_int, c_int, c_int, c_f64, ctypes.POINTER(c_f32), c_int,
                                    ctypes.POINTER(c_int), ctypes.POINTER(c_int), ctypes.POINTER(c_int)]),
    "rdx_resample_batch": (c_int, [c_vp, c_vp, c_vp, ctypes.POINTER(ResampleJob), c_int, c_vp]),
    "rdx_pad_mixup": (c_int, [c_vp, ctypes.POINTER(c_i64), ctypes.POINTER(c_i64), ctypes.POINTER(c_i64), c_int,
                              c_i64, ctypes.POINTER(c_int), c_f32, c_vp, c_vp]),
    "rdx_bnselu_fwd": (c_int, [c_int, c_vp, c_vp, c_vp, c_vp, c_vp, c_vp, c_vp, c_i64, c_int, c_vp]),
    "rdx_bnselu_bwd": (c_int, [c_int, c_vp, c_vp, c_vp, c_vp, c_vp, c_vp, c_vp, c_vp, c_vp, c_i64, c_int, c_vp]),
    "rdx_res_tail_fwd": (c_int, [c_int, c_vp, c_vp, c_vp, c_vp, c_vp, c_i64, c_int, c_int, c_vp]),
    "rdx_res_tail_bwd": (c_int, [c_int, c_vp, c_vp, c_vp, c_vp, c_i64, c_int, c_int, c_vp]),
    "rdx_row_ln_fwd": (c_int, [c_int, c_vp, c_vp, c_vp, c_f32, c_int, c_vp, c_vp, c_vp, c_i64, c_int, c_vp]),
    "rdx_row_ln_bwd": (c_int, [c_int, c_vp, c_int] + [c_vp] * 7 + [c_i64, c_int, c_vp]),
    "rdx_sincnet_b0_fwd": (c_int, [c_vp] * 7 + [c_int, c_int, c_int, c_int, c_vp]),
    "rdx_sincnet_b0_nblk": (c_int, [c_i64]),
    "rdx_sincnet_b0_bwd": (c_int, [c_vp] * 7 + [c_int, c_int, c_int, c_int, c_vp]),
    "rdx_b0x_fwd": (c_int, [c_vp] * 8 + [c_int, c_int, c_int, c_vp]),
    "rdx_b0x_bwd_nblk": (c_int, [c_int, c_int]),
    "rdx_b0x_bwd": (c_int, [c_vp] * 9 + [c_int, c_int, c_int, c_vp]),
    "rdx_posconv_fwd": (c_int, [c_vp] * 5 + [c_int, c_int, c_vp]),
    "rdx_posconv_bwd": (c_int, [c_vp] * 4 + [c_int, c_int, c_vp]),
    "rdx_gemm_bf16": (c_int, [c_vp, c_i64, c_vp, c_i64, c_vp, c_i64, c_int, c_int, c_int, c_vp, c_int, c_vp, c_i64,
                              c_vp, c_i64, c_vp, c_int, c_f32, c_vp]),
    "rdx_wgemm_bf16": (c_int, [c_vp, c_i64, c_vp, c_i64, c_vp, c_i64, c_int, c_int, c_int, c_vp, c_int, c_vp, c_i64,
                               c_vp, c_i64, c_int, c_vp]),
    "rdx_wgemm_pick": (c_int, [c_int, c_int, c_int]),
    "rdx_wgemm_bf16_ex": (c_int, [c_vp, c_i64, c_vp, c_i64, c_vp, c_i64, c_int, c_int, c_int, c_vp, c_int, c_vp,
                                  c_i64, c_vp, c_i64, c_int, c_int, c_vp, c_i64, c_vp, c_i64, c_vp]),
    "rdx_wgemm_ws_bytes": (c_i64, [c_int, c_int, c_int, c_int]),
    "rdx_wgrad_chunk": (c_int, [c_int, c_int, c_int]),
    "rdx_wgrad_ws_floats": (c_i64, [c_int, c_int, c_int]),
    "rdx_wgrad_acc": (c_int, [c_vp, c_i64, c_vp, c_i64, c_int, c_int, c_int, c_vp, c_i64, c_vp, c_vp, c_i64, c_vp]),
    "rdx_wgrad_many_ws_floats": (c_i64, [c_int, c_vp, c_vp, c_vp, c_vp]),
    "rdx_wgrad_acc_many": (c_int, [c_int] + [c_vp] * 10 + [c_vp, c_i64, c_vp]),
    "rdx_adamw_many_max": (c_int, []),
    "rdx_adamw_many": (c_int, [c_int] + [c_vp] * 6 + [c_f64] * 5 + [c_vp, c_vp, c_vp]),
    "rdx_wgemm_counters": (c_i64, [c_int, c_int, c_int]),
    "rdx_sincconv_absmaxpool_f16mfma": (c_int, [c_vp, c_i64, c_i64, c_vp, c_int, c_int, c_int, c_int, c_vp, c_int,
                                                c_vp, c_vp]),
    "rdx_scan2_chunks": (c_int, [c_int]),
    "rdx_scan2_rec_elems": (c_i64, [c_int, c_int, c_int, c_int, c_int]),
    "rdx_scan2_fwd": (c_int, [c_int] + [c_vp] * 5 + [c_i64] + [c_vp] * 6 + [c_int] * 5 + [c_vp]),
    "rdx_scan2_bwd": (c_int, [c_int] + [c_vp] * 5 + [c_i64] + [c_vp] * 5 + [c_i64] + [c_vp] * 6 + [c_i64, c_vp]
                      + [c_int] * 5 + [c_vp]),
    "rdx_pgemm_bf16": (c_int, [c_vp, c_i64, c_vp, c_i64, c_vp, c_i64, c_int, c_int, c_int, c_vp, c_int, c_vp, c_i64,
                               c_vp, c_i64, c_int, c_int, c_vp]),
    "rdx_pgemm_prof": (c_int, [c_vp, c_i64, c_vp, c_i64, c_vp, c_i64, c_int, c_int, c_int, c_vp, c_int, c_int, c_vp,
                               c_vp]),
    "rdx_hgemm": (c_int, [c_vp, c_i64, c_vp, c_i64, c_vp, c_i64, c_int, c_int, c_int, c_vp, c_int, c_vp, c_i64, c_vp,
                          c_i64, c_int, c_int, c_int, c_vp, c_i64, c_vp, c_i64, c_vp]),
    "rdx_hgemm_ws_bytes": (c_i64, [c_int, c_int, c_int, c_int]),
    "rdx_colsum_many": (c_int, [c_int, c_vp, c_vp, c_vp, c_vp, c_vp, c_vp]),
    "rdx_lgemm": (c_int, [c_vp, c_i64, c_int, c_vp, c_i64, c_vp, c_i64, c_int, c_int, c_int, c_int, c_vp, c_int,
                          c_vp, c_i64, c_vp, c_i64, c_vp, c_i64, c_vp]),
    "rdx_hgemm_counters": (c_i64, [c_int, c_int, c_int]),
    "rdx_hgemm_sk_ws_bytes": (c_i64, [c_int, c_int, c_int, c_int]),
    "rdx_gemm_bf16_strided": (c_int, [c_vp, c_i64, c_i64, c_vp, c_i64, c_vp, c_i64, c_i64, c_int, c_int, c_int, c_int,
                                      c_vp, c_vp]),
    "rdx_fe_conv0": (c_int, [c_vp, c_i64, c_i64, c_vp, c_vp, c_vp, c_vp, c_f32, c_int, c_int, c_vp, c_vp]),
    "rdx_fe_ln_gelu": (c_int, [c_vp, c_i64, c_vp, c_vp, c_f32, c_vp, c_vp]),
    "rdx_sconv_dgrad_bnselu": (c_int, [c_vp, c_vp, c_vp, c_vp, c_vp, c_vp, c_int, c_int, c_int, c_int, c_int, c_int,
                                       c_int, c_vp]),
    "rdx_sconv_fwd": (c_int, [c_vp, c_vp, c_vp, c_vp, c_vp, c_int, c_int, c_int, c_int, c_int, c_int, c_int, c_vp]),
    "rdx_sconv_fwd_res": (c_int, [c_vp, c_vp, c_vp, c_vp, c_int, c_int, c_int, c_int, c_int, c_int, c_int, c_vp]),
    "rdx_sconv_fwd_pool": (c_int, [c_vp] * 6 + [c_int] * 5 + [c_vp]),
    "rdx_sconv_fwd_res_pool": (c_int, [c_vp] * 6 + [c_int] * 7 + [c_vp]),
    "rdx_sconv_dgrad_bnselu_pool": (c_int, [c_vp] * 7 + [c_int] * 7 + [c_vp]),
    "rdx_sconv_dgrad_pool": (c_int, [c_vp] * 4 + [c_int] * 7 + [c_vp]),
    "rdx_sconv_wgrad_pool": (c_int, [c_vp] * 5 + [c_int] * 7 + [c_vp]),
    "rdx_sconv_wgrad_nblk": (c_int, [c_int, c_int, c_int]),
    "rdx_sconv_wgrad": (c_int, [c_vp, c_vp, c_vp, c_vp, c_int, c_int, c_int, c_int, c_int, c_int, c_int, c_vp]),
    "rdx_sconv_wprep_many": (c_int, [c_int, c_vp, c_vp, c_vp, c_vp, c_vp, c_vp, c_vp]),
    "rdx_se_fwd": (c_int, [c_vp] * 7 + [c_int] * 4 + [c_vp]),
    "rdx_se_bwd_part_floats": (c_i64, [c_int, c_int, c_int]),
    "rdx_se_bwd": (c_int, [c_vp] * 11 + [c_int] * 4 + [c_vp]),
    "rdx_attn_pool_fwd": (c_int, [c_vp] * 5 + [c_int] * 3 + [c_vp]),
    "rdx_attn_pool_bwd": (c_int, [c_vp] * 8 + [c_int] * 3 + [c_vp]),
    "rdx_upcat_fwd": (c_int, [c_vp] * 3 + [c_int] * 4 + [c_vp]),
    "rdx_upcat_bwd": (c_int, [c_vp] * 2 + [c_int] * 4 + [c_vp]),
    "rdx_attn_fwd": (c_int, [c_vp, c_i64, c_vp, c_i64, c_vp, c_i64, c_vp, c_vp, c_vp, c_int, c_f32, c_f32, c_vp, c_i64,
                             c_vp, c_vp, c_int, c_int, c_int, c_int, c_vp]),
    "rdx_attn_keep_mask_words": (c_i64, [c_int, c_int, c_int]),
    "rdx_attn_bwd": (c_int, [c_vp, c_i64, c_vp, c_i64, c_vp, c_i64, c_vp, c_vp, c_vp, c_int, c_f32, c_f32, c_vp, c_i64,
                             c_vp, c_vp, c_i64, c_vp, c_vp, c_vp, c_vp, c_i64, c_vp, c_int, c_int, c_int, c_int, c_vp]),
    "rdx_attn_bwd_fused": (c_int, [c_vp, c_i64, c_vp, c_i64, c_vp, c_i64, c_vp, c_vp, c_vp, c_f32, c_f32, c_vp, c_i64,
                                   c_vp, c_vp, c_i64, c_vp, c_vp, c_vp, c_vp, c_i64, c_vp, c_int, c_int, c_int, c_int,
                                   c_vp]),
    "rdx_attn_bwd_split_ws": (c_i64, [c_int, c_int]),
    "rdx_attn_bwd_fused_split": (c_int, [c_vp, c_i64, c_vp, c_i64, c_vp, c_i64, c_vp, c_vp, c_vp, c_f32, c_f32, c_vp,
                                         c_i64, c_vp, c_vp, c_i64, c_vp, c_vp, c_vp, c_vp, c_i64, c_vp, c_vp, c_i64,
                                         c_vp, c_i64, c_int, c_int, c_int, c_int, c_vp]),
    "rdx_attn_dropout_mask": (c_int, [c_vp, c_int, c_f32, c_vp, c_i64, c_int, c_vp]),
    "rdx_dropout_mask": (c_int, [c_vp, c_int, c_f32, c_vp, c_i64, c_vp]),
    "rdx_wl_ln1_fwd": (c_int, [c_vp] * 3 + [c_f32] + [c_vp] * 5 + [c_int, c_vp,
                       c_int, c_int, c_f32, c_vp, c_i64] + [c_vp] * 3
                       + [c_i64, c_int, c_vp]),
    "rdx_wl_add_ln_fwd": (c_int, [c_vp, c_vp, c_vp, c_int, c_f32, c_vp, c_vp,
                          c_vp, c_f32, c_vp, c_vp, c_vp, c_i64, c_int,
                          c_vp]),
    "rdx_wl_residual": (c_int, [c_vp, c_vp, c_vp, c_int, c_f32, c_vp, c_i64,
                        c_vp]),
    "rdx_wl_dropout_bwd": (c_int, [c_vp, c_vp, c_int, c_f32, c_vp, c_i64,
                           c_vp]),
    "rdx_wl_gelu": (c_int, [c_int, c_vp, c_vp, c_vp, c_i64, c_vp]),
    "rdx_wl_ln_bwd": (c_int, [c_vp, c_i64] + [c_vp] * 7 + [c_int, c_f32, c_vp,
                      c_i64, c_int, c_vp]),
    "rdx_wl_ln1_bwd": (c_int, [c_vp, c_i64] + [c_vp] * 11 + [c_int, c_vp, c_int,
                       c_int, c_f32, c_vp, c_vp, c_vp, c_i64, c_int, c_vp]),
    "rdx_wl_ln1_bwd_ex": (c_int, [c_vp, c_i64] + [c_vp] * 11 + [c_int, c_vp, c_int, c_int, c_f32] + [c_vp] * 3
                          + [c_vp, c_vp, c_int, c_f32, c_vp, c_i64, c_int, c_vp]),
    "rdx_wl_res_ln1_fwd": (c_int, [c_vp, c_vp, c_int, c_f32, c_vp, c_vp, c_vp, c_f32] + [c_vp] * 5
                           + [c_int, c_vp, c_int, c_int, c_f32, c_vp, c_i64, c_vp, c_vp, c_vp, c_i64, c_int, c_vp]),
    "rdx_wl_lora_grad": (c_int, [c_vp, c_i64, c_vp, c_i64, c_vp, c_i64, c_vp, c_int, c_int, c_f32, c_f32,
                                 c_vp, c_vp, c_vp, c_vp, c_i64, c_int, c_int, c_vp]),
    "rdx_wl_lora_pack": (c_int, [c_int, c_vp, c_vp, c_vp, c_i64, c_int,
                         c_f32, c_int, c_vp]),
    "rdx_timestamp_acc": (c_int, [c_vp, c_int, c_vp]),
    "rdx_wallclock_khz": (c_int, [c_int]),
    "rdx_focal_mixup_fwd": (c_int, [c_vp, c_int, c_int, c_int, c_int, c_vp, c_vp, c_vp, c_int, c_f32, c_f32, c_int,
                                    c_f32, c_vp, c_vp, c_vp]),
    "rdx_focal_mixup_bwd": (c_int, [c_vp, c_vp, c_vp, c_int, c_int, c_vp]),
    "rdx_ocsupcon_eligible": (c_int, [c_vp, c_int, c_int, c_int, c_int]),
    "rdx_ocsupcon_mixup_fwd": (c_int, [c_vp, c_int, c_int, c_int, c_int, c_vp, c_vp, c_vp, c_vp, c_int] + [c_f32] * 7
                               + [c_vp] * 5),
    "rdx_ocsupcon_mixup_bwd": (c_int, [c_vp, c_vp, c_vp, c_int, c_i64, c_vp, c_int, c_int, c_vp, c_vp]),
    "rdx_gat_eligible": (c_int, [c_vp, c_int, c_int, c_int, c_f32]),
    "rdx_gat_att_fwd": (c_int, [c_vp] * 4 + [c_f32] + [c_int] * 4 + [c_vp] * 3),
    "rdx_gat_att_bwd": (c_int, [c_vp] * 5 + [c_f32, c_vp] + [c_int] * 4 + [c_vp] * 5),
    "rdx_hgemm_x3": (c_int, [c_vp, c_vp, c_i64, c_i64, c_vp, c_vp, c_i64, c_vp, c_vp, c_i64, c_i64, c_int, c_int, c_int,
                             c_int, c_vp, c_int, c_int, c_int, c_int, c_vp, c_i64, c_vp, c_i64, c_vp]),
    "rdx_hgemm_batched": (c_int, [c_vp, c_i64, c_i64, c_vp, c_i64, c_vp, c_i64, c_i64, c_int, c_int, c_int, c_int,
                                  c_vp, c_int, c_int, c_vp]),
    "rdx_x3_split": (c_int, [c_vp, c_i64, c_i64, c_int, c_vp, c_vp, c_i64, c_vp]),
    "rdx_x3_ln_split": (c_int, [c_vp, c_vp, c_vp, c_vp, c_vp, c_f32, c_vp, c_vp, c_i64, c_vp, c_vp, c_vp, c_vp, c_vp,
                                c_i64, c_int, c_vp]),
    "rdx_x3_attn_fwd": (c_int, [c_vp, c_vp, c_vp, c_i64, c_vp, c_vp, c_f32, c_vp, c_vp, c_i64, c_int, c_int, c_int,
                                c_int, c_vp]),
    "rdx_x3_posconv_fwd": (c_int, [c_vp, c_vp, c_vp, c_vp, c_vp, c_int, c_int, c_vp]),
    "rdx_x3_fe_conv0": (c_int, [c_vp, c_i64, c_i64, c_vp, c_vp, c_vp, c_vp, c_f32, c_int, c_int, c_vp, c_vp, c_vp]),
    "rdx_x3_fe_ln_gelu": (c_int, [c_vp, c_i64, c_vp, c_vp, c_vp, c_f32, c_vp, c_vp, c_vp, c_vp]),
    "rdx_x3_b0x_fwd": (c_int, [c_vp] * 9 + [c_int, c_int, c_int, c_vp]),
    "rdx_x3_sconv_fwd": (c_int, [c_vp] * 5 + [c_int] * 7 + [c_vp]),
    "rdx_fgm_attack": (c_int, [c_int, ctypes.POINTER(c_vp), ctypes.POINTER(c_vp), ctypes.POINTER(c_vp),
                               ctypes.POINTER(c_i64), c_f32, c_vp, c_vp]),
}

_lock = threading.Lock()
_lib = None
_lib16 = None


def header_symbols():
    import re
    hdr = os.path.join(_HERE, "..", "..", "include", "radhip.h")
    text = open(hdr).read()
    return sorted(set(re.findall(r"^\s*(?:const char\*|int64_t|int)\s+(rdx_\w+)\s*\(", text, re.M)))


def _load(path, mode):
    if not os.path.exists(path):
        raise RuntimeError(
            f"{os.path.basename(path)} not found at {path}: build it with `make -C csrc` "
            "(or __graft_entry__.build()); there is no CPU fallback for the HIP path")
    L = ctypes.CDLL(path, mode=mode)
    for name, (res, args) in SIGNATURES.items():
        fn = getattr(L, name)
        fn.restype = res
        fn.argtypes = args
    return L


def lib():
    global _lib
    if _lib is not None:
        return _lib
    with _lock:
        if _lib is None:
            _lib = _load(LIB_PATH, ctypes.RTLD_GLOBAL)
    return _lib


def lib16():
    global _lib16
    if _lib16 is not None:
        return _lib16
    lib()
    with _lock:
        if _lib16 is None:
            _lib16 = _load(LIB16_PATH, ctypes.RTLD_LOCAL)
    return _lib16


def check(code, what=""):
    if code != 0:
        msg = lib().rdx_strerror(int(code)).decode()
        raise RuntimeError(f"radhip {what} failed: code {code} ({msg})")


def ptr_array(ptrs):
    arr = (c_vp * len(ptrs))()
    for i, p in enumerate(ptrs):
        arr[i] = p
    return arr
```

Before: 510.0 utt/s.

## Split WavLM layernorm rows across multiple waves with M-dependent geometry

Templates the WavLM LayerNorm forward and backward kernels (ln1 fwd, add+ln, ln bwd, ln1 bwd) on waves-per-row and rows-per-block. A row can now be split across 2 or 4 waves with an LDS cross-wave reduction, and elements are laid out in interleaved float4 chunks for coalesced access. A per-kernel table picks the geometry by M, with a runtime override and a policy query exposed through the C API. The goal is more parallelism and better memory coalescing for these row kernels when LoRA is off. The LoRA paths keep one wave per row, and the extra __syncthreads and remapped dropout indices add cost and complexity.

```diff
diff --git a/include/radhip.h b/include/radhip.h
--- a/include/radhip.h
+++ b/include/radhip.h
@@ -209,6 +209,8 @@
                      float* dbq, float* dav, float* dbv, int64_t M, int E, int r, void* stream);
 int rdx_wl_lora_pack(int nl, const float* const* bq, const float* const* bv, void* const* wext, int64_t ldw,
                      int r, float scale, int E, void* stream);
+int rdx_wl_rows_policy(int kernel, int64_t M, int lora, int* waves, int* rows);
+int rdx_wl_rows_override(int waves, int rows);
 
 #define RDX_EPI_BIAS 0
 #define RDX_EPI_BIAS_GELU 1
diff --git a/robust-audio-deepfake-evolution_amd/csrc/wavlm_layer.hip b/robust-audio-deepfake-evolution_amd/csrc/wavlm_layer.hip
--- a/robust-audio-deepfake-evolution_amd/csrc/wavlm_layer.hip
+++ b/robust-audio-deepfake-evolution_amd/csrc/wavlm_layer.hip
@@ -17,73 +17,77 @@
   return drop_keep(seed, idx, d.thr) ? d.inv_keep : 0.f;
 }
 
-__device__ __forceinline__ void load16(const float* p, float* v) {
-  const float4* q = reinterpret_cast<const float4*>(p);
-#pragma unroll
-  for (int i = 0; i < 4; ++i) {
-    float4 t = q[i];
-    v[4 * i] = t.x; v[4 * i + 1] = t.y; v[4 * i + 2] = t.z; v[4 * i + 3] = t.w;
-  }
-}
-__device__ __forceinline__ void store16(float* p, const float* v) {
-  float4* q = reinterpret_cast<float4*>(p);
-#pragma unroll
-  for (int i = 0; i < 4; ++i) q[i] = make_float4(v[4 * i], v[4 * i + 1], v[4 * i + 2], v[4 * i + 3]);
-}
-__device__ __forceinline__ void load16_bf(const hst* p, float* v) {
-  const uint4* q = reinterpret_cast<const uint4*>(p);
-#pragma unroll
-  for (int i = 0; i < 2; ++i) {
-    uint4 t = q[i];
-    uint32_t w[4] = {t.x, t.y, t.z, t.w};
-#pragma unroll
-    for (int j = 0; j < 4; ++j) {
-      v[8 * i + 2 * j] = hlo(w[j]);
-      v[8 * i + 2 * j + 1] = hhi(w[j]);
-    }
-  }
-}
-struct Bf16x16 {
-  uint4 q[2];
+constexpr int WL_CHUNK = 4 * RDX_WAVE;
+__device__ __forceinline__ constexpr int wl_elem(int k) { return (k >> 2) * WL_CHUNK + (k & 3); }
+
+template <int N>
+__device__ __forceinline__ void load_chunks(const float* p, float* v) {
+#pragma unroll
+  for (int j = 0; j < N; ++j) {
+    const float4 t = *reinterpret_cast<const float4*>(p + j * WL_CHUNK);
+    v[4 * j] = t.x; v[4 * j + 1] = t.y; v[4 * j + 2] = t.z; v[4 * j + 3] = t.w;
+  }
+}
+template <int N>
+__device__ __forceinline__ void store_chunks(float* p, const float* v) {
+#pragma unroll
+  for (int j = 0; j < N; ++j)
+    *reinterpret_cast<float4*>(p + j * WL_CHUNK) = make_float4(v[4 * j], v[4 * j + 1], v[4 * j + 2], v[4 * j + 3]);
+}
+template <int N>
+struct HChunks {
+  uint2 q[N];
 };
-__device__ __forceinline__ Bf16x16 load16_bf_raw(const hst* p) {
-  const uint4* q = reinterpret_cast<const uint4*>(p);
-  return Bf16x16{{q[0], q[1]}};
-}
-__device__ __forceinline__ void unpack16_bf(const Bf16x16& t, float* v) {
-#pragma unroll
-  for (int i = 0; i < 2; ++i) {
-    uint32_t w[4] = {t.q[i].x, t.q[i].y, t.q[i].z, t.q[i].w};
-#pragma unroll
-    for (int j = 0; j < 4; ++j) {
-      v[8 * i + 2 * j] = hlo(w[j]);
-      v[8 * i + 2 * j + 1] = hhi(w[j]);
-    }
-  }
-}
-__device__ __forceinline__ void store16_bf(hst* p, const float* v) {
-  uint4* q = reinterpret_cast<uint4*>(p);
-#pragma unroll
-  for (int i = 0; i < 2; ++i) {
-    uint32_t w[4];
-#pragma unroll
-    for (int j = 0; j < 4; ++j) w[j] = hbits(v[8 * i + 2 * j]) | (hbits(v[8 * i + 2 * j + 1]) << 16);
-    q[i] = make_uint4(w[0], w[1], w[2], w[3]);
-  }
-}
-
-__device__ __forceinline__ void row_stats(const float* v, float eps, float& mean, float& rstd) {
+template <int N>
+__device__ __forceinline__ HChunks<N> load_chunks_h_raw(const hst* p) {
+  HChunks<N> t;
+#pragma unroll
+  for (int j = 0; j < N; ++j) t.q[j] = *reinterpret_cast<const uint2*>(p + j * WL_CHUNK);
+  return t;
+}
+template <int N>
+__device__ __forceinline__ void unpack_chunks_h(const HChunks<N>& t, float* v) {
+#pragma unroll
+  for (int j = 0; j < N; ++j) {
+    v[4 * j] = hlo(t.q[j].x);
+    v[4 * j + 1] = hhi(t.q[j].x);
+    v[4 * j + 2] = hlo(t.q[j].y);
+    v[4 * j + 3] = hhi(t.q[j].y);
+  }
+}
+template <int N>
+__device__ __forceinline__ void store_chunks_h(hst* p, const float* v) {
+#pragma unroll
+  for (int j = 0; j < N; ++j)
+    *reinterpret_cast<uint2*>(p + j * WL_CHUNK) =
+        make_uint2(hbits(v[4 * j]) | (hbits(v[4 * j + 1]) << 16), hbits(v[4 * j + 2]) | (hbits(v[4 * j + 3]) << 16));
+}
+
+template <int W>
+__device__ __forceinline__ float row_total(float part, float* slots, int w, int lane) {
+  if (W == 1) return part;
+  if (lane == 0) slots[w] = part;
+  __syncthreads();
+  float t = slots[0];
+#pragma unroll
+  for (int k = 1; k < W; ++k) t += slots[k];
+  return t;
+}
+
+template <int W>
+__device__ __forceinline__ void row_stats(const float* v, float eps, float& mean, float& rstd, float* slots, int w,
+                                          int lane) {
   float s = 0.f;
 #pragma unroll
-  for (int i = 0; i < WL_VPL; ++i) s += v[i];
-  mean = wave_sum(s) * (1.0f / WL_E);
+  for (int i = 0; i < WL_VPL / W; ++i) s += v[i];
+  mean = row_total<W>(wave_sum(s), slots, w, lane) * (1.0f / WL_E);
   float q = 0.f;
 #pragma unroll
-  for (int i = 0; i < WL_VPL; ++i) {
+  for (int i = 0; i < WL_VPL / W; ++i) {
     float d = v[i] - mean;
     q += d * d;
   }
-  rstd = rsqrtf(wave_sum(q) * (1.0f / WL_E) + eps);
+  rstd = rsqrtf(row_total<W>(wave_sum(q), slots + W, w, lane) * (1.0f / WL_E) + eps);
 }
 
 __device__ __forceinline__ float wave_sum16(float* v, int lane) {
@@ -120,20 +124,22 @@
   const float* gconst;
 };
 
-__device__ __forceinline__ void gate_z(const GateW& g, const float* wgp, const float* x, int lane, float* z) {
-  const int part = lane & 3;
-#pragma unroll
-  for (int j = 0; j < 8; ++j) {
-    const float4* w = reinterpret_cast<const float4*>(wgp + j * 64 + part * 16);
-    float acc = 0.f;
-#pragma unroll
-    for (int i = 0; i < 4; ++i) {
-      float4 t = w[i];
-      acc += t.x * x[4 * i] + t.y * x[4 * i + 1] + t.z * x[4 * i + 2] + t.w * x[4 * i + 3];
-    }
-    acc += __shfl_xor(acc, 1, 64);
-    acc += __shfl_xor(acc, 2, 64);
-    z[j] = acc + g.bg[j];
+template <int N>
+__device__ __forceinline__ void gate_z(const GateW& g, const float* wgp, const float* x, int lane, float* za,
+                                       float* zb) {
+  const int d0 = (lane & 15) * 4;
+  float4 w[8];
+#pragma unroll
+  for (int j = 0; j < 8; ++j) w[j] = *reinterpret_cast<const float4*>(wgp + j * 64 + d0);
+  const float ba = g.bg[0] + g.bg[1] + g.bg[2] + g.bg[3], bb = g.bg[4] + g.bg[5] + g.bg[6] + g.bg[7];
+#pragma unroll
+  for (int c = 0; c < N; ++c) {
+    float s[2] = {0.f, 0.f};
+#pragma unroll
+    for (int j = 0; j < 8; ++j)
+      s[j >> 2] += w[j].x * x[4 * c] + w[j].y * x[4 * c + 1] + w[j].z * x[4 * c + 2] + w[j].w * x[4 * c + 3];
+    za[c] = row16_sum(s[0]) + ba;
+    zb[c] = row16_sum(s[1]) + bb;
   }
 }
 
@@ -162,7 +168,6 @@
 #define WL_LN1_ROWS_DEF 4
 #endif
 constexpr int WL_LN1_ROWS = WL_LN1_ROWS_DEF;
-constexpr int WL_LN1_THREADS = WL_LN1_ROWS * RDX_WAVE;
 
 typedef __attribute__((ext_vector_type(4))) int wl_i32x4;
 __device__ void wl_load_lds(wl_i32x4 rsrc, __attribute__((address_space(3))) uint32_t* lds, int size, int voffset,
@@ -176,12 +181,12 @@
   r.w = 0x00020000;
   return r;
 }
-constexpr int WL_A_INSTR = WL_R2 * WL_E * 2 / 1024 / (WL_LN1_THREADS / 64);
-static_assert(WL_A_INSTR * 1024 * (WL_LN1_THREADS / 64) == WL_R2 * WL_E * 2, "whole 1 KB instructions per wave");
-template <bool kLora>
+template <bool kLora, int NW>
 __device__ __forceinline__ void stage_dma(float* swg, hst* sA, const float* wg, const hst* Aq, const hst* Av) {
+  constexpr int WL_A_INSTR = WL_R2 * WL_E * 2 / 1024 / NW;
+  static_assert(!kLora || (NW == WL_LN1_ROWS && WL_A_INSTR % 2 == 0 && WL_A_INSTR * 1024 * NW == WL_R2 * WL_E * 2),
+                "LoRA-A is staged by WL_LN1_ROWS one-wave rows: whole 1 KB instructions, half per adapter");
   const int wv = __builtin_amdgcn_readfirstlane(threadIdx.x >> 6), lane = threadIdx.x & 63;
-  constexpr int NW = WL_LN1_THREADS / 64;
   if (wv == 0) {
     const wl_i32x4 rg = wl_rsrc(wg, 8 * 64 * 4);
 #pragma unroll
@@ -202,61 +207,68 @@
   }
 }
 
-template <bool kLora>
-__global__ __launch_bounds__(WL_LN1_THREADS) void wl_ln1_fwd_kernel(Ln1Args a) {
+template <bool kLora, int W, int R>
+__global__ __launch_bounds__(W * R * RDX_WAVE) void wl_ln1_fwd_kernel(Ln1Args a) {
+  constexpr int N = 4 / W, NV = WL_VPL / W;
   __shared__ __attribute__((aligned(16))) hst sA[kLora ? WL_R2 * WL_E : 8];
   __shared__ __attribute__((aligned(16))) float swg[8 * 64];
-  const int lane = threadIdx.x & 63;
-  const int64_t m = (int64_t)blockIdx.x * WL_LN1_ROWS + (threadIdx.x >> 6);
+  __shared__ float sred[R][2 * W];
+  static_assert(!kLora || W == 1, "the LoRA-active kernels run one wave per row (no geometry measured faster)");
+  const int lane = threadIdx.x & 63, wv = threadIdx.x >> 6, row = wv / W, w = wv % W;
+  const int64_t m = (int64_t)blockIdx.x * R + row;
   const bool live = m < a.M;
-  const int e0 = lane * WL_VPL;
-  float v[WL_VPL], gm[WL_VPL], bt[WL_VPL], dl[WL_VPL];
-  Bf16x16 dlr;
+  const int e0 = w * N * WL_CHUNK + lane * 4;
+  float v[NV], gm[NV], bt[NV], dl[NV];
+  HChunks<N> dlr;
   const uint64_t sr = (a.h2 && a.dres.thr) ? attn_seed(a.dres.seed_dev, a.dres.salt) : 0;
-  stage_dma<kLora>(swg, sA, a.g.wg, a.Aq, a.Av);
+  stage_dma<kLora, W * R>(swg, sA, a.g.wg, a.Aq, a.Av);
   if (live) {
-    load16(a.h2 ? a.h2 + m * WL_E + e0 : a.h + m * WL_E + e0, v);
-    if (a.h2) dlr = load16_bf_raw(a.delta + m * WL_E + e0);
-    load16(a.gamma + e0, gm);
-    load16(a.beta + e0, bt);
+    load_chunks<N>(a.h2 ? a.h2 + m * WL_E + e0 : a.h + m * WL_E + e0, v);
+    if (a.h2) dlr = load_chunks_h_raw<N>(a.delta + m * WL_E + e0);
+    load_chunks<N>(a.gamma + e0, gm);
+    load_chunks<N>(a.beta + e0, bt);
+  } else {
+#pragma unroll
+    for (int i = 0; i < NV; ++i) v[i] = 0.f;
   }
   __builtin_amdgcn_s_waitcnt(0);
   __syncthreads();
+  if (live && a.h2) {
+    unpack_chunks_h<N>(dlr, dl);
+#pragma unroll
+    for (int i = 0; i < NV; ++i)
+      v[i] += dl[i] * (a.dres.thr ? drop_scale(a.dres, sr, (uint64_t)m * WL_E + e0 + wl_elem(i)) : 1.0f);
+    store_chunks<N>(a.hout + m * WL_E + e0, v);
+  }
+  float mean, rstd;
+  row_stats<W>(v, a.eps, mean, rstd, sred[row], w, lane);
   if (live) {
-    if (a.h2) {
-      unpack16_bf(dlr, dl);
-
-#pragma unroll
-      for (int i = 0; i < WL_VPL; ++i)
-        v[i] += dl[i] * (a.dres.thr ? drop_scale(a.dres, sr, (uint64_t)m * WL_E + e0 + i) : 1.0f);
-      store16(a.hout + m * WL_E + e0, v);
-    }
-    float mean, rstd;
-    row_stats(v, a.eps, mean, rstd);
-#pragma unroll
-    for (int i = 0; i < WL_VPL; ++i) v[i] = hround((v[i] - mean) * rstd * gm[i] + bt[i]);
-    store16_bf(a.x1 + m * a.ldx + e0, v);
-    if (lane == 0) {
+#pragma unroll
+    for (int i = 0; i < NV; ++i) v[i] = hround((v[i] - mean) * rstd * gm[i] + bt[i]);
+    store_chunks_h<N>(a.x1 + m * a.ldx + e0, v);
+    if (w == 0 && lane == 0) {
       a.mean[m] = mean;
       a.rstd[m] = rstd;
     }
-    float z[8];
-    gate_z(a.g, swg, v, lane, z);
-    if ((lane & 3) == 0) {
-      const int head = lane >> 2;
-      float ga = sigmoidf_(z[0] + z[1] + z[2] + z[3]);
-      float gb = sigmoidf_(z[4] + z[5] + z[6] + z[7]);
-      a.gate[m * (WL_E / 64) + head] = ga * (gb * a.g.gconst[head] - 1.0f) + 2.0f;
+    float za[N], zb[N];
+    gate_z<N>(a.g, swg, v, lane, za, zb);
+    if ((lane & 15) == 0) {
+#pragma unroll
+      for (int c = 0; c < N; ++c) {
+        const int head = (w * N + c) * 4 + (lane >> 4);
+        const float ga = sigmoidf_(za[c]), gb = sigmoidf_(zb[c]);
+        a.gate[m * (WL_E / 64) + head] = ga * (gb * a.g.gconst[head] - 1.0f) + 2.0f;
+      }
     }
   }
   if (kLora) {
     if (!live) return;
     const uint64_t sq = a.dq.thr ? attn_seed(a.dq.seed_dev, a.dq.salt) : 0;
     const uint64_t sv = a.dv.thr ? attn_seed(a.dv.seed_dev, a.dv.salt) : 0;
-    uint32_t mq[WL_VPL / 2], mv[WL_VPL / 2];
-#pragma unroll
-    for (int j = 0; j < WL_VPL / 2; ++j) {
-      const uint64_t idx = (uint64_t)m * WL_E + e0 + 2 * j;
+    uint32_t mq[NV / 2], mv[NV / 2];
+#pragma unroll
+    for (int j = 0; j < NV / 2; ++j) {
+      const uint64_t idx = (uint64_t)m * WL_E + e0 + wl_elem(2 * j);
       mq[j] = hpack2(v[2 * j] * drop_scale(a.dq, sq, idx), v[2 * j + 1] * drop_scale(a.dq, sq, idx + 1));
       mv[j] = hpack2(v[2 * j] * drop_scale(a.dv, sv, idx), v[2 * j + 1] * drop_scale(a.dv, sv, idx + 1));
     }
@@ -264,15 +276,16 @@
 #pragma unroll
     for (int k = 0; k < WL_R2; ++k) {
       const uint32_t* x = k < WL_R2 / 2 ? mq : mv;
-      const uint4* wp = reinterpret_cast<const uint4*>(sA + k * WL_E + e0);
-      const uint4 w0 = wp[0], w1 = wp[1];
-      const uint32_t w[8] = {w0.x, w0.y, w0.z, w0.w, w1.x, w1.y, w1.z, w1.w};
       float s = 0.f;
 #pragma unroll
-      for (int j = 0; j < WL_VPL / 2; ++j) s = hdot2(w[j], x[j], s);
+      for (int c = 0; c < N; ++c) {
+        const uint2 wk = *reinterpret_cast<const uint2*>(sA + k * WL_E + e0 + c * WL_CHUNK);
+        s = hdot2(wk.x, x[2 * c], s);
+        s = hdot2(wk.y, x[2 * c + 1], s);
+      }
       acc[k] = s;
     }
-    float tot = wave_sum16(acc, lane);
+    const float tot = wave_sum16(acc, lane);
     if ((lane & 3) == 0) a.x1[m * a.ldx + WL_E + sum16_index(lane)] = f2h(tot);
   }
 }
@@ -291,32 +304,43 @@
   int64_t M;
 };
 
-__global__ __launch_bounds__(256) void wl_add_ln_fwd_kernel(AddLnArgs a) {
-  const int lane = threadIdx.x & 63;
-  const int64_t m = (int64_t)blockIdx.x * 4 + (threadIdx.x >> 6);
-  if (m >= a.M) return;
-  const int e0 = lane * WL_VPL;
-  float v[WL_VPL], dl[WL_VPL], gm[WL_VPL], bt[WL_VPL];
-  load16(a.h + m * WL_E + e0, v);
-  const Bf16x16 dlr = load16_bf_raw(a.delta + m * WL_E + e0);
-  load16(a.gamma + e0, gm);
-  load16(a.beta + e0, bt);
-  unpack16_bf(dlr, dl);
-  const uint64_t seed = a.d.thr ? attn_seed(a.d.seed_dev, a.d.salt) : 0;
-#pragma unroll
-  for (int i = 0; i < WL_VPL; ++i)
-    v[i] += dl[i] * (a.d.thr ? drop_scale(a.d, seed, (uint64_t)m * WL_E + e0 + i) : 1.0f);
-  store16(a.h2 + m * WL_E + e0, v);
+template <int W, int R>
+__global__ __launch_bounds__(W * R * RDX_WAVE) void wl_add_ln_fwd_kernel(AddLnArgs a) {
+  constexpr int N = 4 / W, NV = WL_VPL / W;
+  __shared__ float sred[R][2 * W];
+  const int lane = threadIdx.x & 63, wv = threadIdx.x >> 6, row = wv / W, w = wv % W;
+  const int64_t m = (int64_t)blockIdx.x * R + row;
+  const bool live = m < a.M;
+  if (W == 1 && !live) return;
+  const int e0 = w * N * WL_CHUNK + lane * 4;
+  float v[NV], dl[NV], gm[NV], bt[NV];
+  if (live) {
+    load_chunks<N>(a.h + m * WL_E + e0, v);
+    const HChunks<N> dlr = load_chunks_h_raw<N>(a.delta + m * WL_E + e0);
+    load_chunks<N>(a.gamma + e0, gm);
+    load_chunks<N>(a.beta + e0, bt);
+    unpack_chunks_h<N>(dlr, dl);
+    const uint64_t seed = a.d.thr ? attn_seed(a.d.seed_dev, a.d.salt) : 0;
+#pragma unroll
+    for (int i = 0; i < NV; ++i)
+      v[i] += dl[i] * (a.d.thr ? drop_scale(a.d, seed, (uint64_t)m * WL_E + e0 + wl_elem(i)) : 1.0f);
+    store_chunks<N>(a.h2 + m * WL_E + e0, v);
+  } else {
+#pragma unroll
+    for (int i = 0; i < NV; ++i) v[i] = 0.f;
+  }
   float mean, rstd;
-  row_stats(v, a.eps, mean, rstd);
-#pragma unroll
-  for (int i = 0; i < WL_VPL; ++i) v[i] = (v[i] - mean) * rstd * gm[i] + bt[i];
-  store16_bf(a.x + m * WL_E + e0, v);
-  if (lane == 0) {
+  row_stats<W>(v, a.eps, mean, rstd, sred[row], w, lane);
+  if (!live) return;
+#pragma unroll
+  for (int i = 0; i < NV; ++i) v[i] = (v[i] - mean) * rstd * gm[i] + bt[i];
+  store_chunks_h<N>(a.x + m * WL_E + e0, v);
+  if (w == 0 && lane == 0) {
     a.mean[m] = mean;
     a.rstd[m] = rstd;
   }
 }
+
 
 __global__ __launch_bounds__(256) void wl_residual_kernel(const float* __restrict__ h,
                                                           const hst* __restrict__ delta, Drop d,
@@ -402,47 +426,79 @@
   int64_t M;
 };
 
+template <int W>
 __device__ __forceinline__ void ln_bwd_row(const float* dx, const float* x, float mean, float rstd, const float* gm,
-                                           float* out) {
-  float g[WL_VPL], xh[WL_VPL], s1 = 0.f, s2 = 0.f;
-#pragma unroll
-  for (int i = 0; i < WL_VPL; ++i) {
+                                           float* out, float* slots, int w, int lane) {
+  constexpr int NV = WL_VPL / W;
+  float g[NV], xh[NV], s1 = 0.f, s2 = 0.f;
+#pragma unroll
+  for (int i = 0; i < NV; ++i) {
     xh[i] = (x[i] - mean) * rstd;
     g[i] = dx[i] * gm[i];
     s1 += g[i];
     s2 += g[i] * xh[i];
   }
-  s1 = wave_sum(s1) * (1.0f / WL_E);
-  s2 = wave_sum(s2) * (1.0f / WL_E);
-#pragma unroll
-  for (int i = 0; i < WL_VPL; ++i) out[i] = rstd * (g[i] - s1 - xh[i] * s2);
-}
-
-__global__ __launch_bounds__(256) void wl_ln_bwd_kernel(LnBwdArgs a) {
-  const int lane = threadIdx.x & 63;
-  const int64_t m = (int64_t)blockIdx.x * 4 + (threadIdx.x >> 6);
-  if (m >= a.M) return;
-  const int e0 = lane * WL_VPL;
-  float dx[WL_VPL], x[WL_VPL], gm[WL_VPL], o[WL_VPL], r[WL_VPL];
+  s1 = wave_sum(s1);
+  s2 = wave_sum(s2);
+  if (W > 1) {
+    if (lane == 0) {
+      slots[w] = s1;
+      slots[W + w] = s2;
+    }
+    __syncthreads();
+    s1 = slots[0];
+    s2 = slots[W];
+#pragma unroll
+    for (int k = 1; k < W; ++k) {
+      s1 += slots[k];
+      s2 += slots[W + k];
+    }
+  }
+  s1 *= 1.0f / WL_E;
+  s2 *= 1.0f / WL_E;
+#pragma unroll
+  for (int i = 0; i < NV; ++i) out[i] = rstd * (g[i] - s1 - xh[i] * s2);
+}
+
+template <int W, int R>
+__global__ __launch_bounds__(W * R * RDX_WAVE) void wl_ln_bwd_kernel(LnBwdArgs a) {
+  constexpr int N = 4 / W, NV = WL_VPL / W;
+  __shared__ float sred[R][2 * W];
+  const int lane = threadIdx.x & 63, wv = threadIdx.x >> 6, row = wv / W, w = wv % W;
+  const int64_t m = (int64_t)blockIdx.x * R + row;
+  const bool live = m < a.M;
+  if (W == 1 && !live) return;
+  const int e0 = w * N * WL_CHUNK + lane * 4;
+  float dx[NV], x[NV], gm[NV], o[NV], r[NV];
+  float mean = 0.f, rstd = 0.f;
   const uint64_t seed = (a.ddrop && a.d.thr) ? attn_seed(a.d.seed_dev, a.d.salt) : 0;
-  const Bf16x16 dxr = load16_bf_raw(a.dx + m * a.ldd + e0);
-  load16(a.h + m * WL_E + e0, x);
-  load16(a.gamma + e0, gm);
-  if (a.dres) load16(a.dres + m * WL_E + e0, r);
-  unpack16_bf(dxr, dx);
-  ln_bwd_row(dx, x, a.mean[m], a.rstd[m], gm, o);
+  if (live) {
+    const HChunks<N> dxr = load_chunks_h_raw<N>(a.dx + m * a.ldd + e0);
+    load_chunks<N>(a.h + m * WL_E + e0, x);
+    load_chunks<N>(a.gamma + e0, gm);
+    if (a.dres) load_chunks<N>(a.dres + m * WL_E + e0, r);
+    mean = a.mean[m];
+    rstd = a.rstd[m];
+    unpack_chunks_h<N>(dxr, dx);
+  } else {
+#pragma unroll
+    for (int i = 0; i < NV; ++i) dx[i] = x[i] = gm[i] = 0.f;
+  }
+  ln_bwd_row<W>(dx, x, mean, rstd, gm, o, sred[row], w, lane);
+  if (!live) return;
   if (a.dres) {
 #pragma unroll
-    for (int i = 0; i < WL_VPL; ++i) o[i] += r[i];
-  }
-  store16(a.dh + m * WL_E + e0, o);
+    for (int i = 0; i < NV; ++i) o[i] += r[i];
+  }
+  store_chunks<N>(a.dh + m * WL_E + e0, o);
   if (a.ddrop) {
 #pragma unroll
-    for (int i = 0; i < WL_VPL; ++i)
-      o[i] *= a.d.thr ? drop_scale(a.d, seed, (uint64_t)m * WL_E + e0 + i) : 1.0f;
-    store16_bf(a.ddrop + m * WL_E + e0, o);
-  }
-}
+    for (int i = 0; i < NV; ++i)
+      o[i] *= a.d.thr ? drop_scale(a.d, seed, (uint64_t)m * WL_E + e0 + wl_elem(i)) : 1.0f;
+    store_chunks_h<N>(a.ddrop + m * WL_E + e0, o);
+  }
+}
+
 
 struct Ln1BwdArgs {
   const hst* dx1;
@@ -467,117 +523,128 @@
   hst* ddrop;
 };
 
-template <bool kLora>
-__global__ __launch_bounds__(WL_LN1_THREADS) void wl_ln1_bwd_kernel(Ln1BwdArgs a) {
+template <bool kLora, int W, int R>
+__global__ __launch_bounds__(W * R * RDX_WAVE) void wl_ln1_bwd_kernel(Ln1BwdArgs a) {
+  static_assert(!kLora || W == 1, "the LoRA-active kernels run one wave per row");
+  constexpr int N = 4 / W, NV = WL_VPL / W;
   __shared__ __attribute__((aligned(16))) hst sA[kLora ? WL_R2 * WL_E : 8];
   __shared__ __attribute__((aligned(16))) float swg[8 * 64];
-  const int lane = threadIdx.x & 63;
-  const int64_t m = (int64_t)blockIdx.x * WL_LN1_ROWS + (threadIdx.x >> 6);
+  __shared__ float sred[R][2 * W];
+  const int lane = threadIdx.x & 63, wv = threadIdx.x >> 6, row = wv / W, w = wv % W;
+  const int64_t m = (int64_t)blockIdx.x * R + row;
   const bool live = m < a.M;
-  const int e0 = lane * WL_VPL;
-  const int part = lane & 3, head = lane >> 2;
-  float x[WL_VPL], x1[WL_VPL], dx[WL_VPL], r[WL_VPL], sgv[WL_VPL], gm[WL_VPL];
-  float mean = 0.f, rstd = 0.f, dg = 0.f;
-  Bf16x16 dxr;
+  const int e0 = w * N * WL_CHUNK + lane * 4;
+  const int d0 = (lane & 15) * 4, head0 = w * N * 4 + (lane >> 4);
+  float x[NV], x1[NV], dx[NV], r[NV], sgv[NV], gm[NV], dg[N];
+  float mean = 0.f, rstd = 0.f;
+  HChunks<N> dxr;
   const uint64_t sp = (a.ddrop && a.dprev.thr) ? attn_seed(a.dprev.seed_dev, a.dprev.salt) : 0;
-  stage_dma<kLora>(swg, sA, a.g.wg, a.Aq, a.Av);
+  stage_dma<kLora, W * R>(swg, sA, a.g.wg, a.Aq, a.Av);
   if (live) {
-    load16(a.h + m * WL_E + e0, x);
-    dxr = load16_bf_raw(a.dx1 + m * a.ldx + e0);
-    load16(a.dres + m * WL_E + e0, r);
-    if (a.sg) load16(a.sg + m * WL_E + e0, sgv);
-    load16(a.gamma + e0, gm);
-    load16(a.beta + e0, x1);
+    load_chunks<N>(a.h + m * WL_E + e0, x);
+    dxr = load_chunks_h_raw<N>(a.dx1 + m * a.ldx + e0);
+    load_chunks<N>(a.dres + m * WL_E + e0, r);
+    if (a.sg) load_chunks<N>(a.sg + m * WL_E + e0, sgv);
+    load_chunks<N>(a.gamma + e0, gm);
+    load_chunks<N>(a.beta + e0, x1);
     mean = a.mean[m];
     rstd = a.rstd[m];
-    dg = a.dgate[m * (WL_E / 64) + head];
+#pragma unroll
+    for (int c = 0; c < N; ++c) dg[c] = a.dgate[m * (WL_E / 64) + head0 + 4 * c];
   }
   __builtin_amdgcn_s_waitcnt(0);
   __syncthreads();
-  if (!live) return;
-  unpack16_bf(dxr, dx);
-#pragma unroll
-  for (int i = 0; i < WL_VPL; ++i) x1[i] = hround((x[i] - mean) * rstd * gm[i] + x1[i]);
-  float z[8];
-  gate_z(a.g, swg, x1, lane, z);
-  const float ga = sigmoidf_(z[0] + z[1] + z[2] + z[3]), gb = sigmoidf_(z[4] + z[5] + z[6] + z[7]);
-  const float c = a.g.gconst[head];
-  const float dza = dg * (gb * c - 1.0f) * ga * (1.0f - ga);
-  const float dzb = dg * ga * c * gb * (1.0f - gb);
-#pragma unroll 2
-  for (int j = 0; j < 8; ++j) {
-    const float dz = j < 4 ? dza : dzb;
-    const float4* w = reinterpret_cast<const float4*>(swg + j * 64 + part * 16);
-#pragma unroll
-    for (int i = 0; i < 4; ++i) {
-      float4 t = w[i];
-      dx[4 * i] += t.x * dz;
-      dx[4 * i + 1] += t.y * dz;
-      dx[4 * i + 2] += t.z * dz;
-      dx[4 * i + 3] += t.w * dz;
-    }
-  }
-  if (kLora) {
-    const uint64_t sq = a.dq.thr ? attn_seed(a.dq.seed_dev, a.dq.salt) : 0;
-    const uint64_t sv = a.dv.thr ? attn_seed(a.dv.seed_dev, a.dv.salt) : 0;
-    if (a.xd) {
+  if (W == 1 && !live) return;
+  if (live) {
+    unpack_chunks_h<N>(dxr, dx);
+#pragma unroll
+    for (int i = 0; i < NV; ++i) x1[i] = hround((x[i] - mean) * rstd * gm[i] + x1[i]);
+    float za[N], zb[N];
+    gate_z<N>(a.g, swg, x1, lane, za, zb);
+#pragma unroll
+    for (int c = 0; c < N; ++c) {
+      const float ga = sigmoidf_(za[c]), gb = sigmoidf_(zb[c]);
+      const float gc = a.g.gconst[head0 + 4 * c];
+      const float dza = dg[c] * (gb * gc - 1.0f) * ga * (1.0f - ga);
+      const float dzb = dg[c] * ga * gc * gb * (1.0f - gb);
+#pragma unroll
+      for (int j = 0; j < 8; ++j) {
+        const float dz = j < 4 ? dza : dzb;
+        const float4 t = *reinterpret_cast<const float4*>(swg + j * 64 + d0);
+        dx[4 * c] += t.x * dz;
+        dx[4 * c + 1] += t.y * dz;
+        dx[4 * c + 2] += t.z * dz;
+        dx[4 * c + 3] += t.w * dz;
+      }
+    }
+    if (kLora) {
+      const uint64_t sq = a.dq.thr ? attn_seed(a.dq.seed_dev, a.dq.salt) : 0;
+      const uint64_t sv = a.dv.thr ? attn_seed(a.dv.seed_dev, a.dv.salt) : 0;
+      if (a.xd) {
+#pragma unroll
+        for (int which = 0; which < 2; ++which) {
+          const Drop& dd = which ? a.dv : a.dq;
+          const uint64_t sd = which ? sv : sq;
+          float xm[NV];
+#pragma unroll
+          for (int i = 0; i < NV; ++i) xm[i] = x1[i] * drop_scale(dd, sd, (uint64_t)m * WL_E + e0 + wl_elem(i));
+          store_chunks_h<N>(a.xd + (which * a.M + m) * WL_E + e0, xm);
+        }
+      }
+      const uint4 dap[2] = {*reinterpret_cast<const uint4*>(a.dx1 + m * a.ldx + WL_E),
+                            *reinterpret_cast<const uint4*>(a.dx1 + m * a.ldx + WL_E + 8)};
 #pragma unroll
       for (int which = 0; which < 2; ++which) {
+        float acc[NV];
+#pragma unroll
+        for (int i = 0; i < NV; ++i) acc[i] = 0.f;
+        const uint32_t dk[4] = {dap[which].x, dap[which].y, dap[which].z, dap[which].w};
+#pragma unroll
+        for (int kp = 0; kp < WL_R2 / 4; ++kp) {
+          const int k = which * (WL_R2 / 2) + 2 * kp;
+#pragma unroll
+          for (int c = 0; c < N; ++c) {
+            const uint2 ra = *reinterpret_cast<const uint2*>(sA + k * WL_E + e0 + c * WL_CHUNK);
+            const uint2 rb = *reinterpret_cast<const uint2*>(sA + (k + 1) * WL_E + e0 + c * WL_CHUNK);
+            const uint32_t wa[2] = {ra.x, ra.y}, wb[2] = {rb.x, rb.y};
+#pragma unroll
+            for (int j = 0; j < 2; ++j) {
+              const uint32_t ev = __builtin_amdgcn_perm(wb[j], wa[j], 0x05040100u);
+              const uint32_t od = __builtin_amdgcn_perm(wb[j], wa[j], 0x07060302u);
+              acc[4 * c + 2 * j] = hdot2(ev, dk[kp], acc[4 * c + 2 * j]);
+              acc[4 * c + 2 * j + 1] = hdot2(od, dk[kp], acc[4 * c + 2 * j + 1]);
+            }
+          }
+        }
         const Drop& dd = which ? a.dv : a.dq;
         const uint64_t sd = which ? sv : sq;
-        float xm[WL_VPL];
-#pragma unroll
-        for (int i = 0; i < WL_VPL; ++i) xm[i] = x1[i] * drop_scale(dd, sd, (uint64_t)m * WL_E + e0 + i);
-        store16_bf(a.xd + (which * a.M + m) * WL_E + e0, xm);
+#pragma unroll
+        for (int i = 0; i < NV; ++i) dx[i] += acc[i] * drop_scale(dd, sd, (uint64_t)m * WL_E + e0 + wl_elem(i));
       }
     }
-    const uint4 dap[2] = {*reinterpret_cast<const uint4*>(a.dx1 + m * a.ldx + WL_E),
-                          *reinterpret_cast<const uint4*>(a.dx1 + m * a.ldx + WL_E + 8)};
-#pragma unroll
-    for (int which = 0; which < 2; ++which) {
-      float acc[WL_VPL];
-#pragma unroll
-      for (int i = 0; i < WL_VPL; ++i) acc[i] = 0.f;
-      const uint32_t dk[4] = {dap[which].x, dap[which].y, dap[which].z, dap[which].w};
-#pragma unroll
-      for (int kp = 0; kp < WL_R2 / 4; ++kp) {
-        const int k = which * (WL_R2 / 2) + 2 * kp;
-        const uint4* ra = reinterpret_cast<const uint4*>(sA + k * WL_E + e0);
-        const uint4* rb = reinterpret_cast<const uint4*>(sA + (k + 1) * WL_E + e0);
-        const uint4 a0 = ra[0], a1 = ra[1], b0 = rb[0], b1 = rb[1];
-        const uint32_t wa[8] = {a0.x, a0.y, a0.z, a0.w, a1.x, a1.y, a1.z, a1.w};
-        const uint32_t wb[8] = {b0.x, b0.y, b0.z, b0.w, b1.x, b1.y, b1.z, b1.w};
-#pragma unroll
-        for (int j = 0; j < WL_VPL / 2; ++j) {
-          const uint32_t ev = __builtin_amdgcn_perm(wb[j], wa[j], 0x05040100u);
-          const uint32_t od = __builtin_amdgcn_perm(wb[j], wa[j], 0x07060302u);
-          acc[2 * j] = hdot2(ev, dk[kp], acc[2 * j]);
-          acc[2 * j + 1] = hdot2(od, dk[kp], acc[2 * j + 1]);
-        }
-      }
-      const Drop& dd = which ? a.dv : a.dq;
-      const uint64_t sd = which ? sv : sq;
-#pragma unroll
-      for (int i = 0; i < WL_VPL; ++i) dx[i] += acc[i] * drop_scale(dd, sd, (uint64_t)m * WL_E + e0 + i);
-    }
-  }
-  float o[WL_VPL];
-  ln_bwd_row(dx, x, mean, rstd, gm, o);
-#pragma unroll
-  for (int i = 0; i < WL_VPL; ++i) o[i] += r[i];
+  } else {
+#pragma unroll
+    for (int i = 0; i < NV; ++i) dx[i] = x[i] = gm[i] = 0.f;
+  }
+  float o[NV];
+  ln_bwd_row<W>(dx, x, mean, rstd, gm, o, sred[row], w, lane);
+  if (!live) return;
+#pragma unroll
+  for (int i = 0; i < NV; ++i) o[i] += r[i];
   if (a.sg) {
     const float pw = a.sw[0];
 #pragma unroll
-    for (int i = 0; i < WL_VPL; ++i) o[i] = fmaf(pw, sgv[i], o[i]);
-  }
-  store16(a.dh + m * WL_E + e0, o);
+    for (int i = 0; i < NV; ++i) o[i] = fmaf(pw, sgv[i], o[i]);
+  }
+  store_chunks<N>(a.dh + m * WL_E + e0, o);
   if (a.ddrop) {
 #pragma unroll
-    for (int i = 0; i < WL_VPL; ++i)
-      o[i] *= a.dprev.thr ? drop_scale(a.dprev, sp, (uint64_t)m * WL_E + e0 + i) : 1.0f;
-    store16_bf(a.ddrop + m * WL_E + e0, o);
-  }
-}
+    for (int i = 0; i < NV; ++i)
+      o[i] *= a.dprev.thr ? drop_scale(a.dprev, sp, (uint64_t)m * WL_E + e0 + wl_elem(i)) : 1.0f;
+    store_chunks_h<N>(a.ddrop + m * WL_E + e0, o);
+  }
+}
+
 
 constexpr int WL_LG_COLS = 128;
 constexpr int WL_LG_PAD = WL_LG_COLS + 1;
@@ -718,18 +785,55 @@
   return d;
 }
 
-static int blocks_rows(int64_t M) { return (int)((M + 3) / 4); }
-static int blocks_ln1(int64_t M) { return (int)((M + WL_LN1_ROWS - 1) / WL_LN1_ROWS); }
-
-static int ln1_fwd_launch(const Ln1Args& a, bool lora, void* stream) {
-  const int64_t M = a.M;
-  if (lora)
-    hipLaunchKernelGGL(wl_ln1_fwd_kernel<true>, dim3(blocks_ln1(M)), dim3(WL_LN1_THREADS), 0, as_stream(stream), a);
-  else
-    hipLaunchKernelGGL(wl_ln1_fwd_kernel<false>, dim3(blocks_ln1(M)), dim3(WL_LN1_THREADS), 0, as_stream(stream), a);
+struct WlGeo {
+  int w, r;
+};
+enum { WL_K_LN1_FWD = 0, WL_K_ADD_LN = 1, WL_K_LN_BWD = 2, WL_K_LN1_BWD = 3 };
+#ifndef WL_ROWS_SMALL_M
+#define WL_ROWS_SMALL_M 4096
+#endif
+#ifndef WL_GEO_TABLE_DEF
+#define WL_GEO_TABLE_DEF {{{4, 1}, {2, 2}}, {{2, 2}, {2, 2}}, {{2, 2}, {2, 2}}, {{2, 2}, {2, 2}}}
+#endif
+static const WlGeo kWlGeo[4][2] = WL_GEO_TABLE_DEF;
+#define WL_GEOS_LN1_FWD(X) X(1, 4) X(2, 2) X(4, 1)
+#define WL_GEOS(X) X(1, 4) X(2, 2)
+#define WL_GEOS_LORA(X) X(1, 4)
+static_assert(WL_LN1_ROWS == 4, "WL_GEOS_LORA holds (1, WL_LN1_ROWS)");
+
+static WlGeo g_wl_force = {0, 0};
+
+static WlGeo wl_geo(int kernel, int64_t M, bool lora) {
+  if (g_wl_force.w) return g_wl_force;
+  return lora ? WlGeo{1, WL_LN1_ROWS} : kWlGeo[kernel][M >= WL_ROWS_SMALL_M ? 1 : 0];
+}
+static bool wl_geo_built(WlGeo g) {
+#define WL_X(Wv, Rv) if (g.w == Wv && g.r == Rv) return true;
+  WL_GEOS_LN1_FWD(WL_X)
+#undef WL_X
+  return false;
+}
+
+template <typename K, typename A>
+static int wl_launch(K kernel, WlGeo g, const A& a, int64_t M, void* stream) {
+  hipLaunchKernelGGL(kernel, dim3((unsigned)((M + g.r - 1) / g.r)), dim3(g.w * g.r * RDX_WAVE), 0, as_stream(stream), a);
   RDX_LAUNCH_CHECK();
   return 0;
 }
+
+static int ln1_fwd_launch(const Ln1Args& a, bool lora, void* stream) {
+  const WlGeo g = wl_geo(WL_K_LN1_FWD, a.M, lora);
+#define WL_X(Wv, Rv) \
+  if (!lora && g.w == Wv && g.r == Rv) return wl_launch(wl_ln1_fwd_kernel<false, Wv, Rv>, g, a, a.M, stream);
+  WL_GEOS_LN1_FWD(WL_X)
+#undef WL_X
+#define WL_X(Wv, Rv) \
+  if (lora && g.w == Wv && g.r == Rv) return wl_launch(wl_ln1_fwd_kernel<true, Wv, Rv>, g, a, a.M, stream);
+  WL_GEOS_LORA(WL_X)
+#undef WL_X
+  return RDX_EINVAL;
+}
+
 
 
 extern "C" {
@@ -773,8 +877,28 @@
   RDX_REQUIRE(h && delta && h2 && gamma && beta && x && mean && rstd && M > 0 && E == WL_E);
   AddLnArgs a{h, reinterpret_cast<const hst*>(delta), mk_drop(seed_dev, salt, p), h2, gamma, beta, eps,
               reinterpret_cast<hst*>(x), mean, rstd, M};
-  hipLaunchKernelGGL(wl_add_ln_fwd_kernel, dim3(blocks_rows(M)), dim3(256), 0, as_stream(stream), a);
-  RDX_LAUNCH_CHECK();
+  const WlGeo g = wl_geo(WL_K_ADD_LN, M, false);
+#define WL_X(Wv, Rv) if (g.w == Wv && g.r == Rv) return wl_launch(wl_add_ln_fwd_kernel<Wv, Rv>, g, a, M, stream);
+  WL_GEOS(WL_X)
+#undef WL_X
+  return RDX_EINVAL;
+}
+
+int rdx_wl_rows_override(int waves, int rows) {
+  if (waves == 0 && rows == 0) {
+    g_wl_force = WlGeo{0, 0};
+    return 0;
+  }
+  RDX_REQUIRE(wl_geo_built(WlGeo{waves, rows}));
+  g_wl_force = WlGeo{waves, rows};
+  return 0;
+}
+
+int rdx_wl_rows_policy(int kernel, int64_t M, int lora, int* waves, int* rows) {
+  RDX_REQUIRE(kernel >= 0 && kernel < 4 && M > 0 && waves && rows);
+  const WlGeo g = wl_geo(kernel, M, lora != 0);
+  *waves = g.w;
+  *rows = g.r;
   return 0;
 }
 
@@ -816,9 +940,11 @@
   RDX_REQUIRE(dx && h && mean && rstd && gamma && dh && M > 0 && E == WL_E && ldd >= E && ldd % 8 == 0);
   LnBwdArgs a{reinterpret_cast<const hst*>(dx), ldd, h, mean, rstd, gamma, dres, dh,
               mk_drop(seed_dev, salt, p), reinterpret_cast<hst*>(ddrop), M};
-  hipLaunchKernelGGL(wl_ln_bwd_kernel, dim3(blocks_rows(M)), dim3(256), 0, as_stream(stream), a);
-  RDX_LAUNCH_CHECK();
-  return 0;
+  const WlGeo g = wl_geo(WL_K_LN_BWD, M, false);
+#define WL_X(Wv, Rv) if (g.w == Wv && g.r == Rv) return wl_launch(wl_ln_bwd_kernel<Wv, Rv>, g, a, M, stream);
+  WL_GEOS(WL_X)
+#undef WL_X
+  return RDX_EINVAL;
 }
 
 int rdx_wl_ln1_bwd_ex(const void* dx1, int64_t ldx, const float* dgate, const float* h, const float* mean,
@@ -837,12 +963,16 @@
                mk_drop(seed_dev, salt_q, p_lora), mk_drop(seed_dev, salt_v, p_lora),
                dres, dh, reinterpret_cast<hst*>(xd), M, state_grad, state_weight,
                mk_drop(seed_dev, salt_prev, p_prev), reinterpret_cast<hst*>(ddrop_prev)};
-  if (lora)
-    hipLaunchKernelGGL(wl_ln1_bwd_kernel<true>, dim3(blocks_ln1(M)), dim3(WL_LN1_THREADS), 0, as_stream(stream), a);
-  else
-    hipLaunchKernelGGL(wl_ln1_bwd_kernel<false>, dim3(blocks_ln1(M)), dim3(WL_LN1_THREADS), 0, as_stream(stream), a);
-  RDX_LAUNCH_CHECK();
-  return 0;
+  const WlGeo g = wl_geo(WL_K_LN1_BWD, M, lora);
+#define WL_X(Wv, Rv) \
+  if (!lora && g.w == Wv && g.r == Rv) return wl_launch(wl_ln1_bwd_kernel<false, Wv, Rv>, g, a, M, stream);
+  WL_GEOS(WL_X)
+#undef WL_X
+#define WL_X(Wv, Rv) \
+  if (lora && g.w == Wv && g.r == Rv) return wl_launch(wl_ln1_bwd_kernel<true, Wv, Rv>, g, a, M, stream);
+  WL_GEOS_LORA(WL_X)
+#undef WL_X
+  return RDX_EINVAL;
 }
 
 int rdx_wl_ln1_bwd(const void* dx1, int64_t ldx, const float* dgate, const float* h, const float* mean,
diff --git a/robust-audio-deepfake-evolution_amd/radhip/_lib.py b/robust-audio-deepfake-evolution_amd/radhip/_lib.py
--- a/robust-audio-deepfake-evolution_amd/radhip/_lib.py
+++ b/robust-audio-deepfake-evolution_amd/radhip/_lib.py
@@ -191,6 +191,8 @@
                                  c_vp, c_vp, c_vp, c_vp, c_i64, c_int, c_int, c_vp]),
     "rdx_wl_lora_pack": (c_int, [c_int, c_vp, c_vp, c_vp, c_i64, c_int,
                          c_f32, c_int, c_vp]),
+    "rdx_wl_rows_policy": (c_int, [c_int, c_i64, c_int, ctypes.POINTER(c_int), ctypes.POINTER(c_int)]),
+    "rdx_wl_rows_override": (c_int, [c_int, c_int]),
     "rdx_timestamp_acc": (c_int, [c_vp, c_int, c_vp]),
     "rdx_wallclock_khz": (c_int, [c_int]),
     "rdx_focal_mixup_fwd": (c_int, [c_vp, c_int, c_int, c_int, c_int, c_vp, c_vp, c_vp, c_int, c_f32, c_f32, c_int,
```

New measurement: 517.4 utt/s, median of 6. 1.5% higher.
